# alibaba/easydist

Measured on AMD Instinct MI355X. Metric: gpt2_train_samples_per_sec, higher is better.
Workload: dtype bf16; 1 GPU; model=gpt2-small, global_batch=64, seq_len=1024, parallelism=auto(dp1)

## Files before the change

### easydist_amd/ops/csrc/gemm_kernels.hip

```cpp
#include "common.h"
#include "attn_block_map.h"
#include <torch/extension.h>
#include <ATen/cuda/CUDAContext.h>

using f32x4 = __attribute__((ext_vector_type(4))) float;
using bf16x8v = __attribute__((ext_vector_type(8))) __bf16;
using v4s = __attribute__((ext_vector_type(4))) short;
using v8s = __attribute__((ext_vector_type(8))) short;

DEVINL void glds16(const void* gsrc, void* lds_dst) {
  __builtin_amdgcn_global_load_lds(
      (const __attribute__((address_space(1))) unsigned int*)gsrc,
      (__attribute__((address_space(3))) unsigned int*)lds_dst, 16, 0, 0);
}

DEVINL void raw_barrier() { __builtin_amdgcn_s_barrier(); }

#define GELU_C 0.7978845608028654f
#define GELU_A 0.044715f

DEVINL float fast_tanh(float u) {
  return 1.f - 2.f / (__expf(2.f * u) + 1.f);
}

DEVINL float act_apply(int act, float x, float aux) {
  if (act == 1 || act == 3) {
    float u = GELU_C * (x + GELU_A * x * x * x);
    return 0.5f * x * (1.f + fast_tanh(u));
  }
  if (act == 2 || act == 4) {
    float u = GELU_C * (aux + GELU_A * aux * aux * aux);
    float t = fast_tanh(u);
    float d = 0.5f * (1.f + t)
              + 0.5f * aux * (1.f - t * t) * GELU_C
                    * (1.f + 3.f * GELU_A * aux * aux);
    return x * d;
  }
  if (act >= 5) {
    float u = GELU_C * (x + GELU_A * x * x * x);
    return 0.5f * x * (1.f + fast_tanh(u));
  }
  return x;
}

__global__ void __launch_bounds__(256)
gelu_fwd_kernel(const bf16* __restrict__ X, bf16* __restrict__ Y, long n) {
  long i = ((long)blockIdx.x * blockDim.x + threadIdx.x) * 8;
  for (; i + 7 < n; i += (long)gridDim.x * blockDim.x * 8) {
    bf16x8v x = *reinterpret_cast<const bf16x8v*>(&X[i]);
    bf16x8v y;
    #pragma unroll
    for (int e = 0; e < 8; ++e)
      y[e] = (__bf16)act_apply(1, bf2f((bf16)x[e]), 0.f);
    *reinterpret_cast<bf16x8v*>(&Y[i]) = y;
  }
}

__global__ void __launch_bounds__(256)
gelu_bwd_kernel(const bf16* __restrict__ G, const bf16* __restrict__ X,
                bf16* __restrict__ Y, long n) {
  long i = ((long)blockIdx.x * blockDim.x + threadIdx.x) * 8;
  for (; i + 7 < n; i += (long)gridDim.x * blockDim.x * 8) {
    bf16x8v g = *reinterpret_cast<const bf16x8v*>(&G[i]);
    bf16x8v x = *reinterpret_cast<const bf16x8v*>(&X[i]);
    bf16x8v y;
    #pragma unroll
    for (int e = 0; e < 8; ++e)
      y[e] = (__bf16)act_apply(2, bf2f((bf16)g[e]), bf2f((bf16)x[e]));
    *reinterpret_cast<bf16x8v*>(&Y[i]) = y;
  }
}

#define BM 128
#define BN 128
#define BK 32

extern "C" __global__ void __launch_bounds__(256)
gemm_nt_128(const bf16* __restrict__ A, const bf16* __restrict__ Bt,
            bf16* __restrict__ C, const bf16* __restrict__ bias,
            int M, int N, int K) {
  extern __shared__ __attribute__((aligned(16))) char smem[];
  const unsigned ATILE = BM * BK * 2;
  const unsigned BUF = 2 * ATILE;

  unsigned nwg_m = (M + BM - 1) / BM, nwg_n = (N + BN - 1) / BN;
  unsigned wg = xcd_swizzle(blockIdx.x, nwg_m * nwg_n);
  const unsigned m0 = (wg / nwg_n) * BM;
  const unsigned n0 = (wg % nwg_n) * BN;

  const int t = threadIdx.x;
  const int lane = t % WAVE;
  const int wave = t / WAVE;
  const int wm = (wave / 2) * 64;
  const int wn = (wave % 2) * 64;

  auto stage = [&](int buf, int k0) {
    #pragma unroll
    for (int p = 0; p < 2; ++p) {
      int e = (t + p * 256) * 8;
      int row = e / BK, col = e % BK;
      int grow = min((int)m0 + row, M - 1);
      const bf16* src = A + (long)grow * K + k0 + col;
      glds16(src, smem + buf * BUF + (p * 256 + wave * 64) * 16);
    }
    #pragma unroll
    for (int p = 0; p < 2; ++p) {
      int e = (t + p * 256) * 8;
      int row = e / BK, col = e % BK;
      int grow = min((int)n0 + row, N - 1);
      const bf16* src = Bt + (long)grow * K + k0 + col;
      glds16(src, smem + buf * BUF + ATILE + (p * 256 + wave * 64) * 16);
    }
  };

  f32x4 acc[4][4];
  #pragma unroll
  for (int i = 0; i < 4; ++i)
    #pragma unroll
    for (int j = 0; j < 4; ++j)
      acc[i][j] = {0.f, 0.f, 0.f, 0.f};

  stage(0, 0);
  __builtin_amdgcn_s_waitcnt(0);
  __syncthreads();

  const int frag_row = lane & 15;
  const int frag_k = (lane >> 4) * 8;

  int nk = K / BK;
  for (int kt = 0; kt < nk; ++kt) {
    int buf = kt & 1;
    if (kt + 1 < nk) stage(buf ^ 1, (kt + 1) * BK);
    bf16x8v a_frag[4], b_frag[4];
    const char* base = smem;
    #pragma unroll
    for (int i = 0; i < 4; ++i) {
      unsigned off = buf * BUF + ((wm + i * 16 + frag_row) * BK + frag_k) * 2;
      a_frag[i] = *reinterpret_cast<const bf16x8v*>(base + off);
    }
    #pragma unroll
    for (int j = 0; j < 4; ++j) {
      unsigned off = buf * BUF + ATILE +
                     ((wn + j * 16 + frag_row) * BK + frag_k) * 2;
      b_frag[j] = *reinterpret_cast<const bf16x8v*>(base + off);
    }
    #pragma unroll
    for (int i = 0; i < 4; ++i)
      #pragma unroll
      for (int j = 0; j < 4; ++j)
        acc[i][j] = __builtin_amdgcn_mfma_f32_16x16x32_bf16(
            a_frag[i], b_frag[j], acc[i][j], 0, 0, 0);
    __builtin_amdgcn_s_waitcnt(0);
    __syncthreads();
  }

  const int c_col = lane & 15;
  const int c_row0 = (lane >> 4) * 4;
  float bias_v[4] = {0.f, 0.f, 0.f, 0.f};
  if (bias) {
    #pragma unroll
    for (int j = 0; j < 4; ++j)
      bias_v[j] = bf2f(bias[min((int)(n0 + wn + j * 16 + c_col), N - 1)]);
  }
  #pragma unroll
  for (int i = 0; i < 4; ++i) {
    #pragma unroll
    for (int j = 0; j < 4; ++j) {
      #pragma unroll
      for (int reg = 0; reg < 4; ++reg) {
        int gm = m0 + wm + i * 16 + c_row0 + reg;
        int gn = n0 + wn + j * 16 + c_col;
        if (gm < M && gn < N)
          C[(long)gm * N + gn] = f2bf(acc[i][j][reg] + bias_v[j]);
      }
    }
  }
}

#define BM2 256
#define BN2 256
#define BK2 64
#define HALF_B 16384u
#define BUF_B 65536u

template <int SWZ>
DEVINL unsigned sw32(unsigned x) {
  if constexpr (SWZ == 0) return x ^ (((x >> 9) & 1u) << 5);
  else if constexpr (SWZ == 1) return x ^ (((x >> 9) & 3u) << 6);
  else return x ^ (((x >> 8) & 7u) << 4);
}

template <int SWZ>
__global__ void __launch_bounds__(512)
gemm_nt_256(const bf16* __restrict__ A, const bf16* __restrict__ Bt,
            bf16* __restrict__ C, const bf16* __restrict__ bias,
            bf16* __restrict__ aux, int act, int M, int N, int K) {
  extern __shared__ __attribute__((aligned(16))) char smem[];

  unsigned nwg_m = (M + BM2 - 1) / BM2, nwg_n = (N + BN2 - 1) / BN2;
  unsigned wg = xcd_swizzle(blockIdx.x, nwg_m * nwg_n);
  const unsigned m0 = (wg / nwg_n) * BM2;
  const unsigned n0 = (wg % nwg_n) * BN2;

  const int t = threadIdx.x;
  const int lane = t % WAVE;
  const int wave = t / WAVE;
  const int wr = wave >> 2;
  const int wc = wave & 3;

  auto stage_a = [&](int parity, int k0, int h) {
    unsigned dst0 = parity * BUF_B + h * HALF_B;
    #pragma unroll
    for (int i = 0; i < 2; ++i) {
      unsigned p = (i * 512 + t) * 16;
      unsigned L = sw32<SWZ>(p);
      int s = L >> 13;
      int row = (L >> 7) & 63;
      int k = (L & 127) >> 1;
      int grow = min((int)m0 + s * 128 + h * 64 + row, M - 1);
      glds16(A + (long)grow * K + k0 + k,
             smem + dst0 + (i * 512 + wave * 64) * 16);
    }
  };
  auto stage_b = [&](int parity, int k0, int h) {
    unsigned dst0 = parity * BUF_B + 32768u + h * HALF_B;
    #pragma unroll
    for (int i = 0; i < 2; ++i) {
      unsigned p = (i * 512 + t) * 16;
      unsigned L = sw32<SWZ>(p);
      int s = (L >> 12) & 3;
      int col = (L >> 7) & 31;
      int k = (L & 127) >> 1;
      int gcol = min((int)n0 + s * 64 + h * 32 + col, N - 1);
      glds16(Bt + (long)gcol * K + k0 + k,
             smem + dst0 + (i * 512 + wave * 64) * 16);
    }
  };

  const int fr = lane & 15;
  const int fg = lane >> 4;
  auto read_a = [&](bf16x8v (&a)[4][2], int tile, int mh) {
    unsigned base = (tile & 1) * BUF_B + mh * HALF_B;
    #pragma unroll
    for (int i = 0; i < 4; ++i)
      #pragma unroll
      for (int kk = 0; kk < 2; ++kk) {
        unsigned L = wr * 8192u + (i * 16 + fr) * 128u +
                     (kk * 32 + fg * 8) * 2u;
        a[i][kk] = *reinterpret_cast<const bf16x8v*>(smem + base + sw32<SWZ>(L));
      }
  };
  auto read_b = [&](bf16x8v (&b)[2][2], int tile, int nh) {
    unsigned base = (tile & 1) * BUF_B + 32768u + nh * HALF_B;
    #pragma unroll
    for (int j = 0; j < 2; ++j)
      #pragma unroll
      for (int kk = 0; kk < 2; ++kk) {
        unsigned L = wc * 4096u + (j * 16 + fr) * 128u +
                     (kk * 32 + fg * 8) * 2u;
        b[j][kk] = *reinterpret_cast<const bf16x8v*>(smem + base + sw32<SWZ>(L));
      }
  };

  f32x4 acc[8][4];
  #pragma unroll
  for (int i = 0; i < 8; ++i)
    #pragma unroll
    for (int j = 0; j < 4; ++j)
      acc[i][j] = {0.f, 0.f, 0.f, 0.f};

  bf16x8v a_frag[4][2], b_frag[2][2], b0_frag[2][2];
  const int NT = K / BK2;

  auto k_of = [&](int t) { return t < NT ? t * BK2 : 0; };

  stage_a(0, 0, 0); stage_a(0, 0, 1); stage_b(0, 0, 0); stage_b(0, 0, 1);
  stage_a(1, k_of(1), 0); stage_b(1, k_of(1), 1); stage_a(1, k_of(1), 1);
  asm volatile("s_waitcnt vmcnt(6)" ::: "memory");
  raw_barrier();

  auto mfma_quad = [&](int mh, int nh, bf16x8v (&bf)[2][2]) {
    __builtin_amdgcn_s_setprio(1);
    #pragma unroll
    for (int i = 0; i < 4; ++i)
      #pragma unroll
      for (int j = 0; j < 2; ++j)
        #pragma unroll
        for (int kk = 0; kk < 2; ++kk)
          acc[mh * 4 + i][nh * 2 + j] = __builtin_amdgcn_mfma_f32_16x16x32_bf16(
              a_frag[i][kk], bf[j][kk], acc[mh * 4 + i][nh * 2 + j],
              0, 0, 0);
    __builtin_amdgcn_s_setprio(0);
  };

  for (int T = 0; T < NT; ++T) {
    read_a(a_frag, T, 0);
    read_b(b0_frag, T, 0);
    read_b(b_frag, T, 1);
    stage_b((T + 1) & 1, k_of(T + 1), 0);
    mfma_quad(0, 0, b0_frag);
    raw_barrier();
    stage_a(T & 1, k_of(T + 2), 0);
    mfma_quad(0, 1, b_frag);
    raw_barrier();
    read_a(a_frag, T, 1);
    stage_b(T & 1, k_of(T + 2), 1);
    mfma_quad(1, 1, b_frag);
    raw_barrier();
    stage_a(T & 1, k_of(T + 2), 1);
    asm volatile("s_waitcnt vmcnt(6)" ::: "memory");
    mfma_quad(1, 0, b0_frag);
    raw_barrier();
  }

  asm volatile("s_waitcnt vmcnt(0)" ::: "memory");
  raw_barrier();
  bf16* share = reinterpret_cast<bf16*>(smem) + wave * 8192;
  const unsigned wm = wr * 128, wn = wc * 64;
  float bias_v[4] = {0.f, 0.f, 0.f, 0.f};
  if (bias) {
    #pragma unroll
    for (int j = 0; j < 4; ++j)
      bias_v[j] = bf2f(bias[min((int)(n0 + wn + j * 16 + fr), N - 1)]);
  }
  #pragma unroll
  for (int i = 0; i < 8; ++i)
    #pragma unroll
    for (int j = 0; j < 4; ++j)
      #pragma unroll
      for (int r = 0; r < 4; ++r) {
        int row = i * 16 + fg * 4 + r;
        int col = j * 16 + fr;
        share[row * 64 + col] = f2bf(acc[i][j][r] + bias_v[j]);
      }
  lds_fence();
  #pragma unroll
  for (int tt = 0; tt < 16; ++tt) {
    int row = tt * 8 + (lane >> 3);
    int colc = (lane & 7) * 8;
    int gm = m0 + wm + row;
    int gn = n0 + wn + colc;
    if (gm < (int)M && gn + 8 <= (int)N) {
      bf16x8v val = *reinterpret_cast<const bf16x8v*>(&share[row * 64 + colc]);
      if (act) {
        bf16x8v av{};
        if (act == 2 || act == 4)
          av = *reinterpret_cast<const bf16x8v*>(&aux[(long)gm * N + gn]);
        else if (act >= 5)
          *reinterpret_cast<bf16x8v*>(&aux[(long)gm * N + gn]) = val;
        #pragma unroll
        for (int e = 0; e < 8; ++e)
          val[e] = (__bf16)act_apply(act, bf2f((bf16)val[e]),
                                     bf2f((bf16)av[e]));
      }
      *reinterpret_cast<bf16x8v*>(&C[(long)gm * N + gn]) = val;
    } else if (gm < (int)M) {
      for (int e = 0; e < 8 && gn + e < (int)N; ++e) {
        float xv = bf2f(share[row * 64 + colc + e]);
        float axv = (act == 2 || act == 4)
                        ? bf2f(aux[(long)gm * N + gn + e]) : 0.f;
        if (act >= 5) aux[(long)gm * N + gn + e] = f2bf(xv);
        C[(long)gm * N + gn + e] = f2bf(act_apply(act, xv, axv));
      }
    }
  }
}

#define TBR 32
#define TBP 128

DEVINL int tn_unswz(int pos) { return ((pos >> 2) & 1) | ((pos & 3) << 1); }

DEVINL void tn_stage(const bf16* src, long ld, int r0, int p0, int pmax,
                     char* dst_base, int t, int wave) {
  #pragma unroll
  for (int i = 0; i < 2; ++i) {
    unsigned p = (i * 256 + t) * 16;
    int chunk16 = p >> 10;
    unsigned w = p & 1023u;
    int bpos = w >> 7;
    int blk = tn_unswz(bpos);
    int rr = blk * 4 + ((w & 127) >> 5);
    int pp = chunk16 * 16 + ((w & 31) >> 1);
    int gp = min(p0 + pp, pmax - 8);
    glds16(src + (long)(r0 + rr) * ld + gp,
           dst_base + (i * 256 + wave * 64) * 16);
  }
}

DEVINL bf16x8v tn_frag(const char* img, int chunk, int lane) {
  const char* base = img + chunk * 1024 + (lane >> 4) * 128 + (lane & 15) * 8;
  v4s lo = __builtin_amdgcn_ds_read_tr16_b64_v4i16(
      (__attribute__((address_space(3))) v4s*)base);
  v4s hi = __builtin_amdgcn_ds_read_tr16_b64_v4i16(
      (__attribute__((address_space(3))) v4s*)(base + 512));
  v8s out = __builtin_shufflevector(lo, hi, 0, 1, 2, 3, 4, 5, 6, 7);
  return __builtin_bit_cast(bf16x8v, out);
}

extern "C" __global__ void __launch_bounds__(256)
gemm_tn_kernel(const bf16* __restrict__ Ag, const bf16* __restrict__ Bg,
               float* __restrict__ Cw, float* __restrict__ Asum,
               int R, int P, int Q, int splitr) {
  extern __shared__ __attribute__((aligned(16))) char smem[];
  const unsigned IMG = TBR * TBP * 2;
  const unsigned BUF = 2 * IMG;

  unsigned nwg_p = P / TBP, nwg_q = Q / TBP;
  unsigned ntile = nwg_p * nwg_q;
  unsigned wg = xcd_swizzle(blockIdx.x, ntile * splitr);
  unsigned tile = wg / splitr, slice = wg % splitr;
  const unsigned p0 = (tile / nwg_q) * TBP;
  const unsigned q0 = (tile % nwg_q) * TBP;

  int nrt_all = R / TBR;
  int per = (nrt_all + splitr - 1) / splitr;
  int rt0 = slice * per;
  int rt1 = min(nrt_all, rt0 + per);
  if (rt0 >= rt1) return;

  const int t = threadIdx.x;
  const int lane = t % WAVE;
  const int wave = t / WAVE;
  const int wp = (wave >> 1) * 64;
  const int wq = (wave & 1) * 64;

  auto stage = [&](int buf, int rt) {
    tn_stage(Ag, P, rt * TBR, p0, P, smem + buf * BUF, t, wave);
    tn_stage(Bg, Q, rt * TBR, q0, Q, smem + buf * BUF + IMG, t, wave);
  };

  f32x4 acc[4][4];
  float asum_acc[4] = {0.f, 0.f, 0.f, 0.f};
  #pragma unroll
  for (int i = 0; i < 4; ++i)
    #pragma unroll
    for (int j = 0; j < 4; ++j)
      acc[i][j] = {0.f, 0.f, 0.f, 0.f};

  stage(0, rt0);
  __builtin_amdgcn_s_waitcnt(0);
  __syncthreads();
  for (int rt = rt0; rt < rt1; ++rt) {
    int buf = (rt - rt0) & 1;
    if (rt + 1 < rt1) stage(buf ^ 1, rt + 1);
    bf16x8v a_frag[4], b_frag[4];
    #pragma unroll
    for (int i = 0; i < 4; ++i)
      a_frag[i] = tn_frag(smem + buf * BUF, (wp >> 4) + i, lane);
    if (Asum && q0 == 0 && (wave & 1) == 0) {
      #pragma unroll
      for (int i = 0; i < 4; ++i) {
        float acc_s = 0.f;
        #pragma unroll
        for (int u = 0; u < 8; ++u) acc_s += bf2f((bf16)a_frag[i][u]);
        asum_acc[i] += acc_s;
      }
    }
    #pragma unroll
    for (int j = 0; j < 4; ++j)
      b_frag[j] = tn_frag(smem + buf * BUF + IMG, (wq >> 4) + j, lane);
    #pragma unroll
    for (int i = 0; i < 4; ++i)
      #pragma unroll
      for (int j = 0; j < 4; ++j)
        acc[i][j] = __builtin_amdgcn_mfma_f32_16x16x32_bf16(
            a_frag[i], b_frag[j], acc[i][j], 0, 0, 0);
    __builtin_amdgcn_s_waitcnt(0);
    __syncthreads();
  }

  if (Asum && q0 == 0 && (wave & 1) == 0) {
    #pragma unroll
    for (int i = 0; i < 4; ++i) {
      float v = asum_acc[i];
      v += __shfl_down(v, 32, WAVE);
      v += __shfl_down(v, 16, WAVE);
      if (lane < 16) {
        int gp = p0 + wp + i * 16 + lane;
        if (gp < P) atomicAdd(&Asum[gp], v);
      }
    }
  }
  const int c_col = lane & 15;
  const int c_row0 = (lane >> 4) * 4;
  #pragma unroll
  for (int i = 0; i < 4; ++i)
    #pragma unroll
    for (int j = 0; j < 4; ++j)
      #pragma unroll
      for (int reg = 0; reg < 4; ++reg) {
        int gp = p0 + wp + i * 16 + c_row0 + reg;
        int gq = q0 + wq + j * 16 + c_col;
        if (gp < P && gq < Q) {
          if (splitr == 1)
            Cw[(long)gp * Q + gq] = acc[i][j][reg];
          else
            atomicAdd(&Cw[(long)gp * Q + gq], acc[i][j][reg]);
        }
      }
}

#define TBP2 256

DEVINL void tn_stage2(const bf16* src, long ld, int r0, int p0, int pmax,
                      char* dst_base, int t, int wave) {
  #pragma unroll
  for (int i = 0; i < 2; ++i) {
    unsigned p = (i * 512 + t) * 16;
    int chunk16 = p >> 10;
    unsigned w = p & 1023u;
    int bpos = w >> 7;
    int blk = tn_unswz(bpos);
    int rr = blk * 4 + ((w & 127) >> 5);
    int pp = chunk16 * 16 + ((w & 31) >> 1);
    int gp = min(p0 + pp, pmax - 8);
    glds16(src + (long)(r0 + rr) * ld + gp,
           dst_base + (i * 512 + wave * 64) * 16);
  }
}

extern "C" __global__ void __launch_bounds__(512)
gemm_tn_256_kernel(const bf16* __restrict__ Ag, const bf16* __restrict__ Bg,
                   float* __restrict__ Cw, float* __restrict__ Asum,
                   int R, int P, int Q, int splitr) {
  extern __shared__ __attribute__((aligned(16))) char smem[];
  const unsigned IMG = TBR * TBP2 * 2;
  const unsigned BUF = 2 * IMG;

  unsigned nwg_p = (P + TBP2 - 1) / TBP2, nwg_q = (Q + TBP2 - 1) / TBP2;
  unsigned ntile = nwg_p * nwg_q;
  unsigned wg = xcd_swizzle(blockIdx.x, ntile * splitr);
  unsigned tile = wg / splitr, slice = wg % splitr;
  const unsigned p0 = (tile / nwg_q) * TBP2;
  const unsigned q0 = (tile % nwg_q) * TBP2;

  int nrt_all = R / TBR;
  int per = (nrt_all + splitr - 1) / splitr;
  int rt0 = slice * per;
  int rt1 = min(nrt_all, rt0 + per);
  if (rt0 >= rt1) return;

  const int t = threadIdx.x;
  const int lane = t % WAVE;
  const int wave = t / WAVE;
  const int wp = (wave >> 1) * 64;
  const int wq = (wave & 1) * 128;

  auto stage = [&](int buf, int rt) {
    tn_stage2(Ag, P, rt * TBR, p0, P, smem + buf * BUF, t, wave);
    tn_stage2(Bg, Q, rt * TBR, q0, Q, smem + buf * BUF + IMG, t, wave);
  };

  f32x4 acc[4][8];
  float asum_acc[4] = {0.f, 0.f, 0.f, 0.f};
  #pragma unroll
  for (int i = 0; i < 4; ++i)
    #pragma unroll
    for (int j = 0; j < 8; ++j)
      acc[i][j] = {0.f, 0.f, 0.f, 0.f};

  stage(0, rt0);
  __builtin_amdgcn_s_waitcnt(0);
  __syncthreads();
  for (int rt = rt0; rt < rt1; ++rt) {
    int buf = (rt - rt0) & 1;
    if (rt + 1 < rt1) stage(buf ^ 1, rt + 1);
    bf16x8v a_frag[4], b_frag[8];
    #pragma unroll
    for (int i = 0; i < 4; ++i)
      a_frag[i] = tn_frag(smem + buf * BUF, (wp >> 4) + i, lane);
    if (Asum && q0 == 0 && (wave & 1) == 0) {
      #pragma unroll
      for (int i = 0; i < 4; ++i) {
        float acc_s = 0.f;
        #pragma unroll
        for (int u = 0; u < 8; ++u) acc_s += bf2f((bf16)a_frag[i][u]);
        asum_acc[i] += acc_s;
      }
    }
    #pragma unroll
    for (int j = 0; j < 8; ++j)
      b_frag[j] = tn_frag(smem + buf * BUF + IMG, (wq >> 4) + j, lane);
    #pragma unroll
    for (int i = 0; i < 4; ++i)
      #pragma unroll
      for (int j = 0; j < 8; ++j)
        acc[i][j] = __builtin_amdgcn_mfma_f32_16x16x32_bf16(
            a_frag[i], b_frag[j], acc[i][j], 0, 0, 0);
    __builtin_amdgcn_s_waitcnt(0);
    __syncthreads();
  }

  if (Asum && q0 == 0 && (wave & 1) == 0) {
    #pragma unroll
    for (int i = 0; i < 4; ++i) {
      float v = asum_acc[i];
      v += __shfl_down(v, 32, WAVE);
      v += __shfl_down(v, 16, WAVE);
      if (lane < 16) {
        int gp = p0 + wp + i * 16 + lane;
        if (gp < P) atomicAdd(&Asum[gp], v);
      }
    }
  }
  const int c_col = lane & 15;
  const int c_row0 = (lane >> 4) * 4;
  #pragma unroll
  for (int i = 0; i < 4; ++i)
    #pragma unroll
    for (int j = 0; j < 8; ++j)
      #pragma unroll
      for (int reg = 0; reg < 4; ++reg) {
        int gp = p0 + wp + i * 16 + c_row0 + reg;
        int gq = q0 + wq + j * 16 + c_col;
        if (gp < P && gq < Q) {
          if (splitr == 1)
            Cw[(long)gp * Q + gq] = acc[i][j][reg];
          else
            atomicAdd(&Cw[(long)gp * Q + gq], acc[i][j][reg]);
        }
      }
}

at::Tensor gemm_nt_act(const at::Tensor& a, const at::Tensor& bt,
                       const std::optional<at::Tensor>& bias, int64_t act,
                       const std::optional<at::Tensor>& aux) {
  TORCH_CHECK(a.dtype() == at::kBFloat16 && bt.dtype() == at::kBFloat16);
  TORCH_CHECK(a.is_contiguous() && bt.is_contiguous(),
              "gemm_nt wants K-contiguous operands");
  const long M = a.size(0), K = a.size(1), N = bt.size(0);
  TORCH_CHECK(bt.size(1) == K);
  TORCH_CHECK(K % BK == 0, "gemm_nt: K must be a multiple of 32");
  TORCH_CHECK(N % 8 == 0, "gemm_nt: N must be a multiple of 8");
  auto c = at::empty({M, N}, a.options());
  auto stream = at::cuda::getCurrentCUDAStream();
  const bf16* bias_p = bias ? (const bf16*)bias->data_ptr() : nullptr;
  if (K % BK2 == 0 && M >= BM2 && N >= 128) {
    unsigned nwg = ((M + BM2 - 1) / BM2) * ((N + BN2 - 1) / BN2);
    static int swz = []() {
      const char* e = getenv("EASYDIST_NT256_SWZ");
      return e ? atoi(e) : 2;
    }();
    auto kern = swz == 0 ? gemm_nt_256<0> : swz == 2 ? gemm_nt_256<2>
                                          : gemm_nt_256<1>;
    bf16* aux_p = aux ? (bf16*)aux->data_ptr() : nullptr;
    TORCH_CHECK(act == 0 || !(act >= 2) || aux_p,
                "gemm_nt: activation modes 2/4/5/6 need aux");
    hipLaunchKernelGGL(kern, dim3(nwg), dim3(512), 2 * BUF_B, stream,
        (const bf16*)a.data_ptr(), (const bf16*)bt.data_ptr(),
        (bf16*)c.data_ptr(), bias_p, aux_p, (int)act, (int)M, (int)N,
        (int)K);
  } else {
    unsigned nwg = ((M + BM - 1) / BM) * ((N + BN - 1) / BN);
    size_t lds = 2 * 2 * BM * BK * 2;
    hipLaunchKernelGGL(gemm_nt_128, dim3(nwg), dim3(256), lds, stream,
        (const bf16*)a.data_ptr(), (const bf16*)bt.data_ptr(),
        (bf16*)c.data_ptr(), bias_p, (int)M, (int)N, (int)K);
    if (act) {
      if (act == 1) c = at::gelu(c, "tanh");
      else if (act == 3) c = at::gelu(c);
      else if (act == 2) c = at::gelu_backward(c, aux.value(), "tanh");
      else if (act == 4) c = at::gelu_backward(c, aux.value(), "none");
      else if (act >= 5) {
        aux.value().copy_(c);
        c = at::gelu(c, "tanh");
      }
    }
  }
  return c;
}

at::Tensor gemm_nt(const at::Tensor& a, const at::Tensor& bt,
                   const std::optional<at::Tensor>& bias) {
  return gemm_nt_act(a, bt, bias, 0, std::nullopt);
}

at::Tensor gelu_fast(const at::Tensor& x) {
  TORCH_CHECK(x.dtype() == at::kBFloat16 && x.is_contiguous());
  const long n = x.numel();
  TORCH_CHECK(n % 8 == 0, "gelu_fast: numel multiple of 8");
  auto y = at::empty_like(x);
  long thr = n / 8;
  unsigned grid = (unsigned)std::min<long>((thr + 255) / 256, 8192);
  auto stream = at::cuda::getCurrentCUDAStream();
  hipLaunchKernelGGL(gelu_fwd_kernel, dim3(grid), dim3(256), 0, stream,
                     (const bf16*)x.data_ptr(), (bf16*)y.data_ptr(), n);
  return y;
}

at::Tensor gelu_bwd_fast(const at::Tensor& g, const at::Tensor& x) {
  TORCH_CHECK(g.dtype() == at::kBFloat16 && g.is_contiguous());
  TORCH_CHECK(x.dtype() == at::kBFloat16 && x.is_contiguous());
  const long n = x.numel();
  TORCH_CHECK(g.numel() == n && n % 8 == 0);
  auto y = at::empty_like(x);
  long thr = n / 8;
  unsigned grid = (unsigned)std::min<long>((thr + 255) / 256, 8192);
  auto stream = at::cuda::getCurrentCUDAStream();
  hipLaunchKernelGGL(gelu_bwd_kernel, dim3(grid), dim3(256), 0, stream,
                     (const bf16*)g.data_ptr(), (const bf16*)x.data_ptr(),
                     (bf16*)y.data_ptr(), n);
  return y;
}

std::tuple<at::Tensor, at::Tensor>
gemm_nt_gelu(const at::Tensor& a, const at::Tensor& bt,
             const std::optional<at::Tensor>& bias, bool tanh_approx) {
  const long M = a.size(0), K = a.size(1), N = bt.size(0);
  if (K % BK2 == 0 && M >= BM2 && N >= 128) {
    auto pre = at::empty({M, N}, a.options());
    auto act = gemm_nt_act(a, bt, bias, tanh_approx ? 5 : 6, pre);
    return {act, pre};
  }
  auto pre = gemm_nt_act(a, bt, bias, 0, std::nullopt);
  auto act = at::gelu(pre, tanh_approx ? "tanh" : "none");
  return {act, pre};
}

std::tuple<at::Tensor, at::Tensor> gemm_tn_asum(const at::Tensor& a,
                                                const at::Tensor& b);

static at::Tensor tn_launch(const at::Tensor& a, const at::Tensor& b,
                            float* asum_p) {
  TORCH_CHECK(a.dtype() == at::kBFloat16 && b.dtype() == at::kBFloat16);
  TORCH_CHECK(a.is_contiguous() && b.is_contiguous());
  const long R = a.size(0), P = a.size(1), Q = b.size(0) == R ? b.size(1) : -1;
  TORCH_CHECK(Q > 0, "gemm_tn: reduce dims must match");
  TORCH_CHECK(R % TBR == 0, "gemm_tn: R must be a multiple of 32");
  TORCH_CHECK(P % TBP == 0 && Q % TBP == 0,
              "gemm_tn: P, Q must be multiples of 128");
  static int use256 = []() {
    const char* e = getenv("EASYDIST_TN256");
    return e ? atoi(e) : 1;
  }();
  bool big = use256 && R / TBR >= 64 && P >= TBP2 && Q >= TBP2;
  unsigned ntile;
  int splitr = 1;
  if (big) {
    ntile = ((P + TBP2 - 1) / TBP2) * ((Q + TBP2 - 1) / TBP2);
    static int target = []() {
      const char* e = getenv("EASYDIST_TN256_TARGET");
      return e ? atoi(e) : 256;
    }();
    splitr = std::max(1, target / (int)ntile);
    splitr = std::min((long)splitr, R / TBR / 8);
    splitr = std::max(1, std::min(splitr, 64));
  } else {
    ntile = (P / TBP) * (Q / TBP);
    while (ntile * splitr < 512 && splitr < 16 &&
           (R / TBR) % (splitr * 2) == 0 && (R / TBR) / (splitr * 2) >= 1)
      splitr *= 2;
  }
  auto cw = splitr == 1
      ? at::empty({P, Q}, a.options().dtype(at::kFloat))
      : at::zeros({P, Q}, a.options().dtype(at::kFloat));
  auto stream = at::cuda::getCurrentCUDAStream();
  if (big) {
    size_t lds = 2 * 2 * TBR * TBP2 * 2;
    hipLaunchKernelGGL(gemm_tn_256_kernel, dim3(ntile * splitr), dim3(512),
        lds, stream,
        (const bf16*)a.data_ptr(), (const bf16*)b.data_ptr(),
        cw.data_ptr<float>(), asum_p, (int)R, (int)P, (int)Q, splitr);
  } else {
    size_t lds = 2 * 2 * TBR * TBP * 2;
    hipLaunchKernelGGL(gemm_tn_kernel, dim3(ntile * splitr), dim3(256), lds,
        stream,
        (const bf16*)a.data_ptr(), (const bf16*)b.data_ptr(),
        cw.data_ptr<float>(), asum_p, (int)R, (int)P, (int)Q, splitr);
  }
  return cw;
}

at::Tensor gemm_tn(const at::Tensor& a, const at::Tensor& b) {
  return tn_launch(a, b, nullptr).to(at::kBFloat16);
}

std::tuple<at::Tensor, at::Tensor> gemm_tn_asum(const at::Tensor& a,
                                                const at::Tensor& b) {
  auto asum = at::zeros({a.size(1)}, a.options().dtype(at::kFloat));
  auto cw = tn_launch(a, b, asum.data_ptr<float>());
  return {cw.to(at::kBFloat16), asum};
}
```

### easydist_amd/ops/csrc/norm_kernels.hip

```cpp
#include "common.h"
#include <string>
#include <cstdlib>

template <typename T, bool RMS>
__global__ void norm_fwd_kernel(const T* __restrict__ x,
                                const T* __restrict__ w,
                                const T* __restrict__ b,
                                T* __restrict__ out,
                                float* __restrict__ mean_out,
                                float* __restrict__ rstd_out,
                                int rows, int D, float eps) {
  const int wave_id = (blockIdx.x * blockDim.x + threadIdx.x) / WAVE;
  const int lane = threadIdx.x % WAVE;
  if (wave_id >= rows) return;
  const T* xrow = x + (long)wave_id * D;
  T* orow = out + (long)wave_id * D;

  const int VEC = 8;
  float s1 = 0.f, s2 = 0.f;
  for (int i = lane * VEC; i < D; i += WAVE * VEC) {
    bf16x8 xv = *reinterpret_cast<const bf16x8*>(&xrow[i]);
    #pragma unroll
    for (int j = 0; j < VEC; ++j) {
      float f = bf2f(xv.v[j]);
      s1 += f;
      s2 += f * f;
    }
  }
  s1 = wave_sum(s1);
  s2 = wave_sum(s2);
  float mean, rstd;
  if (RMS) {
    mean = 0.f;
    rstd = rsqrtf(s2 / D + eps);
  } else {
    mean = s1 / D;
    rstd = rsqrtf(fmaxf(s2 / D - mean * mean, 0.f) + eps);
  }
  if (lane == 0) {
    if (!RMS) mean_out[wave_id] = mean;
    rstd_out[wave_id] = rstd;
  }
  for (int i = lane * VEC; i < D; i += WAVE * VEC) {
    bf16x8 xv = *reinterpret_cast<const bf16x8*>(&xrow[i]);
    bf16x8 ov;
    bf16x8 wv, bv;
    if (w) wv = *reinterpret_cast<const bf16x8*>(&w[i]);
    if (b) bv = *reinterpret_cast<const bf16x8*>(&b[i]);
    #pragma unroll
    for (int j = 0; j < VEC; ++j) {
      float f = (bf2f(xv.v[j]) - mean) * rstd;
      if (w) f *= bf2f(wv.v[j]);
      if (b) f += bf2f(bv.v[j]);
      ov.v[j] = f2bf(f);
    }
    *reinterpret_cast<bf16x8*>(&orow[i]) = ov;
  }
}

template <bool RMS>
__global__ void norm_fwd_kernel_f32(const float* __restrict__ x,
                                    const float* __restrict__ w,
                                    const float* __restrict__ b,
                                    float* __restrict__ out,
                                    float* __restrict__ mean_out,
                                    float* __restrict__ rstd_out,
                                    int rows, int D, float eps) {
  const int wave_id = (blockIdx.x * blockDim.x + threadIdx.x) / WAVE;
  const int lane = threadIdx.x % WAVE;
  if (wave_id >= rows) return;
  const float* xrow = x + (long)wave_id * D;
  float* orow = out + (long)wave_id * D;
  const int VEC = 4;
  float s1 = 0.f, s2 = 0.f;
  for (int i = lane * VEC; i < D; i += WAVE * VEC) {
    float4 xv = *reinterpret_cast<const float4*>(&xrow[i]);
    s1 += xv.x + xv.y + xv.z + xv.w;
    s2 += xv.x * xv.x + xv.y * xv.y + xv.z * xv.z + xv.w * xv.w;
  }
  s1 = wave_sum(s1);
  s2 = wave_sum(s2);
  float mean, rstd;
  if (RMS) {
    mean = 0.f;
    rstd = rsqrtf(s2 / D + eps);
  } else {
    mean = s1 / D;
    rstd = rsqrtf(fmaxf(s2 / D - mean * mean, 0.f) + eps);
  }
  if (lane == 0) {
    if (!RMS) mean_out[wave_id] = mean;
    rstd_out[wave_id] = rstd;
  }
  for (int i = lane * VEC; i < D; i += WAVE * VEC) {
    float4 xv = *reinterpret_cast<const float4*>(&xrow[i]);
    float4 ov;
    float* xp = &xv.x;
    float* op = &ov.x;
    #pragma unroll
    for (int j = 0; j < VEC; ++j) {
      float f = (xp[j] - mean) * rstd;
      if (w) f *= w[i + j];
      if (b) f += b[i + j];
      op[j] = f;
    }
    *reinterpret_cast<float4*>(&orow[i]) = ov;
  }
}

template <typename T, bool RMS>
__global__ void norm_bwd_kernel(const T* __restrict__ grad,
                                const T* __restrict__ x,
                                const float* __restrict__ mean,
                                const float* __restrict__ rstd,
                                const T* __restrict__ w,
                                T* __restrict__ dx,
                                float* __restrict__ dw,
                                float* __restrict__ db,
                                int rows, int D) {
  const int wave_id = (blockIdx.x * blockDim.x + threadIdx.x) / WAVE;
  const int lane = threadIdx.x % WAVE;
  if (wave_id >= rows) return;
  const T* grow = grad + (long)wave_id * D;
  const T* xrow = x + (long)wave_id * D;
  T* dxrow = dx + (long)wave_id * D;
  const float m = RMS ? 0.f : mean[wave_id];
  const float r = rstd[wave_id];

  const int VEC = 8;
  float sum_gw = 0.f, sum_gwx = 0.f;
  for (int i = lane * VEC; i < D; i += WAVE * VEC) {
    bf16x8 gv = *reinterpret_cast<const bf16x8*>(&grow[i]);
    bf16x8 xv = *reinterpret_cast<const bf16x8*>(&xrow[i]);
    bf16x8 wv;
    if (w) wv = *reinterpret_cast<const bf16x8*>(&w[i]);
    #pragma unroll
    for (int j = 0; j < VEC; ++j) {
      float g = bf2f(gv.v[j]);
      float xh = (bf2f(xv.v[j]) - m) * r;
      float gw = w ? g * bf2f(wv.v[j]) : g;
      sum_gw += gw;
      sum_gwx += gw * xh;
    }
  }
  sum_gw = wave_sum(sum_gw) / D;
  sum_gwx = wave_sum(sum_gwx) / D;
  for (int i = lane * VEC; i < D; i += WAVE * VEC) {
    bf16x8 gv = *reinterpret_cast<const bf16x8*>(&grow[i]);
    bf16x8 xv = *reinterpret_cast<const bf16x8*>(&xrow[i]);
    bf16x8 wv;
    if (w) wv = *reinterpret_cast<const bf16x8*>(&w[i]);
    bf16x8 dxv;
    #pragma unroll
    for (int j = 0; j < VEC; ++j) {
      float g = bf2f(gv.v[j]);
      float xh = (bf2f(xv.v[j]) - m) * r;
      float gw = w ? g * bf2f(wv.v[j]) : g;
      float v = RMS ? r * (gw - xh * sum_gwx)
                    : r * (gw - sum_gw - xh * sum_gwx);
      dxv.v[j] = f2bf(v);
    }
    *reinterpret_cast<bf16x8*>(&dxrow[i]) = dxv;
  }
}

template <typename T, bool RMS>
__global__ void norm_param_grads_kernel(const T* __restrict__ grad,
                                        const T* __restrict__ x,
                                        const float* __restrict__ mean,
                                        const float* __restrict__ rstd,
                                        float* __restrict__ dw,
                                        float* __restrict__ db,
                                        int rows, int D, int rows_per_blk) {
  const int col0 = (blockIdx.x * blockDim.x + threadIdx.x) * 8;
  if (col0 >= D) return;
  const int r0 = blockIdx.y * rows_per_blk;
  const int r1 = min(r0 + rows_per_blk, rows);
  float sw[8] = {0, 0, 0, 0, 0, 0, 0, 0};
  float sb[8] = {0, 0, 0, 0, 0, 0, 0, 0};
  for (int r = r0; r < r1; ++r) {
    const bf16x8 g8 = *reinterpret_cast<const bf16x8*>(
        &grad[(long)r * D + col0]);
    const bf16x8 x8 = *reinterpret_cast<const bf16x8*>(
        &x[(long)r * D + col0]);
    const float m = RMS ? 0.f : mean[r];
    const float rs = rstd[r];
    #pragma unroll
    for (int u = 0; u < 8; ++u) {
      float g = bf2f(g8.v[u]);
      sw[u] += g * (bf2f(x8.v[u]) - m) * rs;
      sb[u] += g;
    }
  }
  #pragma unroll
  for (int u = 0; u < 8; ++u) {
    atomicAdd(&dw[col0 + u], sw[u]);
    atomicAdd(&db[col0 + u], sb[u]);
  }
}

template <typename T, bool RMS>
__global__ void norm_param_grads_scalar_kernel(const T* __restrict__ grad,
                                               const T* __restrict__ x,
                                               const float* __restrict__ mean,
                                               const float* __restrict__ rstd,
                                               float* __restrict__ dw,
                                               float* __restrict__ db,
                                               int rows, int D,
                                               int rows_per_blk) {
  const int col = blockIdx.x * blockDim.x + threadIdx.x;
  if (col >= D) return;
  const int r0 = blockIdx.y * rows_per_blk;
  const int r1 = min(r0 + rows_per_blk, rows);
  float sw = 0.f, sb = 0.f;
  #pragma unroll 8
  for (int r = r0; r < r1; ++r) {
    float g = bf2f(grad[(long)r * D + col]);
    float m = RMS ? 0.f : mean[r];
    float xh = (bf2f(x[(long)r * D + col]) - m) * rstd[r];
    sw += g * xh;
    sb += g;
  }
  atomicAdd(&dw[col], sw);
  atomicAdd(&db[col], sb);
}

static bool lnpg_scalar() {
  static int v = [] {
    const char* e = getenv("EASYDIST_LNPG");
    return (e && std::string(e) == "vector") ? 0 : 1;
  }();
  return v;
}

#include <torch/extension.h>
#include <ATen/cuda/CUDAContext.h>

static void check_lastdim(const at::Tensor& x) {
  TORCH_CHECK(x.is_contiguous(), "norm kernels need contiguous input");
  TORCH_CHECK(x.size(-1) % 8 == 0, "feature dim must be a multiple of 8");
}

static void check_affine(const at::Tensor& x,
                         const std::optional<at::Tensor>& w,
                         const std::optional<at::Tensor>& b) {
  if (w) TORCH_CHECK(w->numel() == x.size(-1), "weight/feature mismatch");
  if (b) TORCH_CHECK(b->numel() == x.size(-1), "bias/feature mismatch");
}

std::tuple<at::Tensor, at::Tensor, at::Tensor>
layer_norm_fwd(const at::Tensor& x, const std::optional<at::Tensor>& w,
               const std::optional<at::Tensor>& b, double eps) {
  check_lastdim(x);
  check_affine(x, w, b);
  const int D = x.size(-1);
  const long rows = x.numel() / D;
  auto out = at::empty_like(x);
  auto stat_shape = x.sizes().vec();
  stat_shape.back() = 1;
  auto mean = at::empty(stat_shape, x.options().dtype(at::kFloat));
  auto rstd = at::empty(stat_shape, x.options().dtype(at::kFloat));
  auto stream = at::cuda::getCurrentCUDAStream();
  const int WPB = 4;
  dim3 block(WAVE * WPB), grid((rows + WPB - 1) / WPB);
  if (x.scalar_type() == at::kBFloat16) {
    hipLaunchKernelGGL((norm_fwd_kernel<bf16, false>), grid, block, 0, stream,
        (const bf16*)x.data_ptr(), w ? (const bf16*)w->data_ptr() : nullptr,
        b ? (const bf16*)b->data_ptr() : nullptr, (bf16*)out.data_ptr(),
        mean.data_ptr<float>(), rstd.data_ptr<float>(), rows, D, (float)eps);
  } else {
    hipLaunchKernelGGL((norm_fwd_kernel_f32<false>), grid, block, 0, stream,
        x.data_ptr<float>(), w ? w->data_ptr<float>() : nullptr,
        b ? b->data_ptr<float>() : nullptr, out.data_ptr<float>(),
        mean.data_ptr<float>(), rstd.data_ptr<float>(), rows, D, (float)eps);
  }
  return {out, mean, rstd};
}

std::tuple<at::Tensor, at::Tensor, at::Tensor>
layer_norm_bwd(const at::Tensor& grad, const at::Tensor& x,
               const at::Tensor& mean, const at::Tensor& rstd,
               const std::optional<at::Tensor>& w,
               std::vector<bool> mask) {
  check_lastdim(x);
  check_affine(x, w, std::nullopt);
  TORCH_CHECK(grad.sizes() == x.sizes() && grad.is_contiguous());
  TORCH_CHECK(mean.numel() == x.numel() / x.size(-1));
  TORCH_CHECK(x.scalar_type() == at::kBFloat16,
              "layer_norm_bwd kernel: bf16 only (fp32 falls back to aten)");
  const int D = x.size(-1);
  const long rows = x.numel() / D;
  auto dx = at::empty_like(x);
  auto dwf = at::zeros({D}, x.options().dtype(at::kFloat));
  auto dbf = at::zeros({D}, x.options().dtype(at::kFloat));
  auto stream = at::cuda::getCurrentCUDAStream();
  const int WPB = 4;
  dim3 block(WAVE * WPB), grid((rows + WPB - 1) / WPB);
  hipLaunchKernelGGL((norm_bwd_kernel<bf16, false>), grid, block, 0, stream,
      (const bf16*)grad.data_ptr(), (const bf16*)x.data_ptr(),
      mean.data_ptr<float>(), rstd.data_ptr<float>(),
      w ? (const bf16*)w->data_ptr() : nullptr, (bf16*)dx.data_ptr(),
      dwf.data_ptr<float>(), dbf.data_ptr<float>(), rows, D);
  const int gx = (D + 511) / 512;
  int rows_per_blk = 256;
  while ((long)gx * ((rows + rows_per_blk - 1) / rows_per_blk) > 1024)
    rows_per_blk *= 2;
  dim3 gblock(64), ggrid(gx, (rows + rows_per_blk - 1) / rows_per_blk);
  if (lnpg_scalar()) {
    const int rpb2 = 256;
    dim3 sb2(256), sg2((D + 255) / 256, (rows + rpb2 - 1) / rpb2);
    hipLaunchKernelGGL((norm_param_grads_scalar_kernel<bf16, false>), sg2,
        sb2, 0, stream, (const bf16*)grad.data_ptr(),
        (const bf16*)x.data_ptr(), mean.data_ptr<float>(),
        rstd.data_ptr<float>(), dwf.data_ptr<float>(),
        dbf.data_ptr<float>(), rows, D, rpb2);
    auto dtype0 = at::kFloat;
    return {dx, dwf.to(dtype0), dbf.to(dtype0)};
  }
  hipLaunchKernelGGL((norm_param_grads_kernel<bf16, false>), ggrid, gblock, 0,
      stream, (const bf16*)grad.data_ptr(), (const bf16*)x.data_ptr(),
      mean.data_ptr<float>(), rstd.data_ptr<float>(), dwf.data_ptr<float>(),
      dbf.data_ptr<float>(), rows, D, rows_per_blk);
  auto dtype = at::kFloat;
  return {dx, dwf.to(dtype), dbf.to(dtype)};
}

std::tuple<at::Tensor, at::Tensor>
rms_norm_fwd(const at::Tensor& x, const std::optional<at::Tensor>& w,
             double eps) {
  check_lastdim(x);
  check_affine(x, w, std::nullopt);
  const int D = x.size(-1);
  const long rows = x.numel() / D;
  auto out = at::empty_like(x);
  auto stat_shape = x.sizes().vec();
  stat_shape.back() = 1;
  auto rstd = at::empty(stat_shape, x.options().dtype(at::kFloat));
  auto stream = at::cuda::getCurrentCUDAStream();
  const int WPB = 4;
  dim3 block(WAVE * WPB), grid((rows + WPB - 1) / WPB);
  if (x.scalar_type() == at::kBFloat16) {
    hipLaunchKernelGGL((norm_fwd_kernel<bf16, true>), grid, block, 0, stream,
        (const bf16*)x.data_ptr(), w ? (const bf16*)w->data_ptr() : nullptr,
        nullptr, (bf16*)out.data_ptr(), nullptr, rstd.data_ptr<float>(),
        rows, D, (float)eps);
  } else {
    hipLaunchKernelGGL((norm_fwd_kernel_f32<true>), grid, block, 0, stream,
        x.data_ptr<float>(), w ? w->data_ptr<float>() : nullptr, nullptr,
        out.data_ptr<float>(), nullptr, rstd.data_ptr<float>(), rows, D,
        (float)eps);
  }
  return {out, rstd};
}

std::tuple<at::Tensor, at::Tensor>
rms_norm_bwd(const at::Tensor& grad, const at::Tensor& x,
             const at::Tensor& rstd, const std::optional<at::Tensor>& w) {
  check_lastdim(x);
  check_affine(x, w, std::nullopt);
  TORCH_CHECK(grad.sizes() == x.sizes() && grad.is_contiguous());
  TORCH_CHECK(x.scalar_type() == at::kBFloat16, "rms_norm_bwd: bf16 only");
  const int D = x.size(-1);
  const long rows = x.numel() / D;
  auto dx = at::empty_like(x);
  auto dwf = at::zeros({D}, x.options().dtype(at::kFloat));
  auto dbf = at::zeros({D}, x.options().dtype(at::kFloat));
  auto stream = at::cuda::getCurrentCUDAStream();
  const int WPB = 4;
  dim3 block(WAVE * WPB), grid((rows + WPB - 1) / WPB);
  hipLaunchKernelGGL((norm_bwd_kernel<bf16, true>), grid, block, 0, stream,
      (const bf16*)grad.data_ptr(), (const bf16*)x.data_ptr(), nullptr,
      rstd.data_ptr<float>(), w ? (const bf16*)w->data_ptr() : nullptr,
      (bf16*)dx.data_ptr(), dwf.data_ptr<float>(), dbf.data_ptr<float>(),
      rows, D);
  const int gx = (D + 511) / 512;
  int rows_per_blk = 256;
  while ((long)gx * ((rows + rows_per_blk - 1) / rows_per_blk) > 1024)
    rows_per_blk *= 2;
  dim3 gblock(64), ggrid(gx, (rows + rows_per_blk - 1) / rows_per_blk);
  hipLaunchKernelGGL((norm_param_grads_kernel<bf16, true>), ggrid, gblock, 0,
      stream, (const bf16*)grad.data_ptr(), (const bf16*)x.data_ptr(),
      nullptr, rstd.data_ptr<float>(), dwf.data_ptr<float>(),
      dbf.data_ptr<float>(), rows, D, rows_per_blk);
  auto dtype = at::kFloat;
  return {dx, dwf.to(dtype)};
}
```

### easydist_amd/ops/csrc/optim_kernels.hip

```cpp
#include "common.h"
#include <torch/extension.h>
#include <ATen/cuda/CUDAContext.h>
#include <ATen/cuda/CUDAGraphsUtils.cuh>
#include <map>
#include <utility>
#include <vector>

struct AdamChunk {
  const float* p;
  const void* g;
  const float* ea;
  const float* eas;
  float* out_p;
  float* out_ea;
  float* out_eas;
  int tensor_idx;
  int n;
};

DEVINL void load_g4(const void* g, int i, int g_bf16, float* out) {
  if (g_bf16) {
    bf16x8 v = *reinterpret_cast<const bf16x8*>(&((const bf16*)g)[i & ~7]);
    const int o = i & 4;
    #pragma unroll
    for (int j = 0; j < 4; ++j) out[j] = bf2f(v.v[o + j]);
  } else {
    float4 v = *reinterpret_cast<const float4*>(&((const float*)g)[i]);
    out[0] = v.x; out[1] = v.y; out[2] = v.z; out[3] = v.w;
  }
}

#define CHUNK_ELEMS 65536

struct StagingPair {
  at::Tensor pinned, dev;
  size_t capacity = 0;
  hipEvent_t h2d_done = nullptr;
};

static StagingPair& staging_for(std::map<std::pair<size_t, const void*>,
                                         StagingPair>& pool,
                                size_t bytes, const void* key_ptr,
                                const at::Device& dev, bool capturing,
                                const char* who) {
  auto& st = pool[{bytes, key_ptr}];
  if (bytes > st.capacity) {
    TORCH_CHECK(!capturing, who,
                ": staging buffers must be warmed up (one eager call per "
                "parameter bank) before hipGraph capture");
    st.pinned = at::empty({(long)bytes},
                          at::TensorOptions().dtype(at::kByte)
                              .pinned_memory(true));
    st.dev = at::empty({(long)bytes},
                       at::TensorOptions().dtype(at::kByte).device(dev));
    st.capacity = bytes;
  }
  if (st.h2d_done == nullptr)
    C10_CUDA_CHECK(hipEventCreateWithFlags(&st.h2d_done,
                                           hipEventDisableTiming));
  else if (!capturing)
    C10_CUDA_CHECK(hipEventSynchronize(st.h2d_done));
  return st;
}

static void staging_finish(std::map<std::pair<size_t, const void*>,
                                    StagingPair>& pool,
                           size_t bytes, const void* key_ptr,
                           bool capturing, hipStream_t stream) {
  auto it = pool.find({bytes, key_ptr});
  if (it == pool.end()) return;
  if (capturing) {
    static std::vector<at::Tensor> keepalive;
    keepalive.push_back(it->second.pinned);
    keepalive.push_back(it->second.dev);
    pool.erase(it);
  } else {
    C10_CUDA_CHECK(hipEventRecord(it->second.h2d_done, stream));
  }
}

__global__ void fused_adam_kernel(const AdamChunk* __restrict__ chunks,
                                  int n_chunks, int g_bf16,
                                  const float* __restrict__ steps,
                                  float lr, float beta1, float beta2,
                                  float weight_decay, float eps) {
  const int c = blockIdx.x;
  if (c >= n_chunks) return;
  const AdamChunk ch = chunks[c];
  const float step = steps[ch.tensor_idx] + 1.f;
  const float bc1 = 1.f - __powf(beta1, step);
  const float bc2 = 1.f - __powf(beta2, step);
  const float inv_bc1 = 1.f / bc1;
  const float rsqrt_bc2 = rsqrtf(bc2);
  #pragma unroll 4
  for (int i = threadIdx.x * 4; i + 3 < ch.n; i += blockDim.x * 4) {
    float4 p = *reinterpret_cast<const float4*>(&ch.p[i]);
    float gg[4];
    load_g4(ch.g, i, g_bf16, gg);
    float4 ea = *reinterpret_cast<const float4*>(&ch.ea[i]);
    float4 eas = *reinterpret_cast<const float4*>(&ch.eas[i]);
    float* pp = &p.x; float* ee = &ea.x; float* ss = &eas.x;
    #pragma unroll
    for (int j = 0; j < 4; ++j) {
      float grad = gg[j];
      if (weight_decay != 0.f) grad += weight_decay * pp[j];
      float m = beta1 * ee[j] + (1.f - beta1) * grad;
      float v = beta2 * ss[j] + (1.f - beta2) * grad * grad;
      float denom = __fsqrt_rn(v) * rsqrt_bc2 + eps;
      pp[j] = pp[j] - lr * (m * inv_bc1) / denom;
      ee[j] = m;
      ss[j] = v;
    }
    *reinterpret_cast<float4*>(&ch.out_p[i]) = p;
    *reinterpret_cast<float4*>(&ch.out_ea[i]) = ea;
    *reinterpret_cast<float4*>(&ch.out_eas[i]) = eas;
  }
  int tail_start = (ch.n / 4) * 4;
  for (int i = tail_start + threadIdx.x; i < ch.n; i += blockDim.x) {
    float grad = g_bf16 ? bf2f(((const bf16*)ch.g)[i])
                        : ((const float*)ch.g)[i];
    if (weight_decay != 0.f) grad += weight_decay * ch.p[i];
    float m = beta1 * ch.ea[i] + (1.f - beta1) * grad;
    float v = beta2 * ch.eas[i] + (1.f - beta2) * grad * grad;
    float denom = __fsqrt_rn(v) * rsqrt_bc2 + eps;
    ch.out_p[i] = ch.p[i] - lr * (m * inv_bc1) / denom;
    ch.out_ea[i] = m;
    ch.out_eas[i] = v;
  }
}

__global__ void bump_steps_kernel(const float* const* __restrict__ in_steps,
                                  float* const* __restrict__ out_steps,
                                  int n) {
  int i = blockIdx.x * blockDim.x + threadIdx.x;
  if (i < n) out_steps[i][0] = in_steps[i][0] + 1.f;
}

std::tuple<std::vector<at::Tensor>, std::vector<at::Tensor>,
           std::vector<at::Tensor>, std::vector<at::Tensor>>
fused_adam_step(std::vector<at::Tensor> params, std::vector<at::Tensor> grads,
                std::vector<at::Tensor> exp_avgs,
                std::vector<at::Tensor> exp_avg_sqs,
                std::vector<at::Tensor> steps, double lr, double beta1,
                double beta2, double weight_decay, double eps) {
  const int T = params.size();
  std::vector<at::Tensor> out_p, out_ea, out_eas, out_steps;
  out_p.reserve(T); out_ea.reserve(T); out_eas.reserve(T);
  const bool g_bf16 = !grads.empty()
      && grads[0].scalar_type() == at::kBFloat16;
  for (int t = 0; t < T; ++t) {
    TORCH_CHECK(params[t].scalar_type() == at::kFloat, "fp32 params only");
    TORCH_CHECK(grads[t].scalar_type()
                    == (g_bf16 ? at::kBFloat16 : at::kFloat),
                "grads must be uniformly fp32 or bf16");
    TORCH_CHECK(params[t].is_contiguous() && grads[t].is_contiguous());
    out_p.push_back(at::empty_like(params[t]));
    out_ea.push_back(at::empty_like(exp_avgs[t]));
    out_eas.push_back(at::empty_like(exp_avg_sqs[t]));
    out_steps.push_back(at::empty_like(steps[t]));
  }
  auto steps_flat = at::empty({T}, params[0].options());
  {
    std::vector<at::Tensor> svec;
    for (auto& s : steps) svec.push_back(s.reshape({1}).to(at::kFloat));
    at::cat_out(steps_flat, svec, 0);
  }

  std::vector<AdamChunk> chunks;
  for (int t = 0; t < T; ++t) {
    long n = params[t].numel();
    for (long off = 0; off < n; off += CHUNK_ELEMS) {
      AdamChunk c;
      c.p = params[t].data_ptr<float>() + off;
      c.g = g_bf16 ? (const void*)((const bf16*)grads[t].data_ptr() + off)
                   : (const void*)(grads[t].data_ptr<float>() + off);
      c.ea = exp_avgs[t].data_ptr<float>() + off;
      c.eas = exp_avg_sqs[t].data_ptr<float>() + off;
      c.out_p = out_p[t].data_ptr<float>() + off;
      c.out_ea = out_ea[t].data_ptr<float>() + off;
      c.out_eas = out_eas[t].data_ptr<float>() + off;
      c.tensor_idx = t;
      c.n = (int)std::min<long>(CHUNK_ELEMS, n - off);
      chunks.push_back(c);
    }
  }
  static std::map<std::pair<size_t, const void*>, StagingPair> g_pool;
  const size_t bytes = chunks.size() * sizeof(AdamChunk);
  const void* key = params[0].data_ptr();
  bool capturing = at::cuda::currentStreamCaptureStatusMayInitCtx() !=
                   at::cuda::CaptureStatus::None;
  auto& st = staging_for(g_pool, bytes, key, params[0].device(), capturing,
                         "fused_adam_step");
  memcpy(st.pinned.data_ptr(), chunks.data(), bytes);
  auto stream = at::cuda::getCurrentCUDAStream();
  C10_CUDA_CHECK(hipMemcpyAsync(st.dev.data_ptr(), st.pinned.data_ptr(),
                                bytes, hipMemcpyHostToDevice, stream));
  hipLaunchKernelGGL(fused_adam_kernel, dim3(chunks.size()), dim3(256), 0,
      stream, (const AdamChunk*)st.dev.data_ptr(), (int)chunks.size(),
      (int)g_bf16, steps_flat.data_ptr<float>(), (float)lr, (float)beta1,
      (float)beta2, (float)weight_decay, (float)eps);
  staging_finish(g_pool, bytes, key, capturing, stream);
  for (int t = 0; t < T; ++t)
    out_steps[t] = steps[t] + 1;
  return {out_p, out_ea, out_eas, out_steps};
}

struct SgdChunk {
  const float* p;
  const void* g;
  const float* buf;
  float* out_p;
  float* out_buf;
  int n;
};

__global__ void fused_sgd_kernel(const SgdChunk* __restrict__ chunks,
                                 int n_chunks, int g_bf16, float lr,
                                 float momentum, float dampening,
                                 float weight_decay, int nesterov) {
  const int c = blockIdx.x;
  if (c >= n_chunks) return;
  const SgdChunk ch = chunks[c];
  for (int i = threadIdx.x; i < ch.n; i += blockDim.x) {
    float grad = g_bf16 ? bf2f(((const bf16*)ch.g)[i])
                        : ((const float*)ch.g)[i];
    if (weight_decay != 0.f) grad += weight_decay * ch.p[i];
    float upd = grad;
    if (momentum != 0.f) {
      float nb = momentum * ch.buf[i] + (1.f - dampening) * grad;
      ch.out_buf[i] = nb;
      upd = nesterov ? grad + momentum * nb : nb;
    }
    ch.out_p[i] = ch.p[i] - lr * upd;
  }
}

std::tuple<std::vector<at::Tensor>, std::vector<at::Tensor>>
fused_sgd_step(std::vector<at::Tensor> params, std::vector<at::Tensor> grads,
               std::vector<at::Tensor> bufs, double lr, double momentum,
               double dampening, double weight_decay, bool nesterov) {
  const int T = params.size();
  const bool has_m = momentum != 0.0;
  TORCH_CHECK(!has_m || (int)bufs.size() == T,
              "momentum needs one buffer per param");
  std::vector<at::Tensor> out_p, out_buf;
  out_p.reserve(T);
  const bool g_bf16 = !grads.empty()
      && grads[0].scalar_type() == at::kBFloat16;
  for (int t = 0; t < T; ++t) {
    TORCH_CHECK(params[t].scalar_type() == at::kFloat, "fp32 params only");
    TORCH_CHECK(grads[t].scalar_type()
                    == (g_bf16 ? at::kBFloat16 : at::kFloat),
                "grads must be uniformly fp32 or bf16");
    TORCH_CHECK(params[t].is_contiguous() && grads[t].is_contiguous());
    out_p.push_back(at::empty_like(params[t]));
    if (has_m) out_buf.push_back(at::empty_like(bufs[t]));
  }
  std::vector<SgdChunk> chunks;
  for (int t = 0; t < T; ++t) {
    long n = params[t].numel();
    for (long off = 0; off < n; off += CHUNK_ELEMS) {
      SgdChunk c;
      c.p = params[t].data_ptr<float>() + off;
      c.g = g_bf16 ? (const void*)((const bf16*)grads[t].data_ptr() + off)
                   : (const void*)(grads[t].data_ptr<float>() + off);
      c.buf = has_m ? bufs[t].data_ptr<float>() + off : nullptr;
      c.out_p = out_p[t].data_ptr<float>() + off;
      c.out_buf = has_m ? out_buf[t].data_ptr<float>() + off : nullptr;
      c.n = (int)std::min<long>(CHUNK_ELEMS, n - off);
      chunks.push_back(c);
    }
  }
  static std::map<std::pair<size_t, const void*>, StagingPair> g_pool;
  const size_t bytes = chunks.size() * sizeof(SgdChunk);
  const void* key = params[0].data_ptr();
  bool capturing = at::cuda::currentStreamCaptureStatusMayInitCtx() !=
                   at::cuda::CaptureStatus::None;
  auto& st = staging_for(g_pool, bytes, key, params[0].device(), capturing,
                         "fused_sgd_step");
  memcpy(st.pinned.data_ptr(), chunks.data(), bytes);
  auto stream = at::cuda::getCurrentCUDAStream();
  C10_CUDA_CHECK(hipMemcpyAsync(st.dev.data_ptr(), st.pinned.data_ptr(),
                                bytes, hipMemcpyHostToDevice, stream));
  hipLaunchKernelGGL(fused_sgd_kernel, dim3(chunks.size()), dim3(256), 0,
      stream, (const SgdChunk*)st.dev.data_ptr(), (int)chunks.size(),
      (int)g_bf16, (float)lr, (float)momentum, (float)dampening,
      (float)weight_decay, nesterov ? 1 : 0);
  staging_finish(g_pool, bytes, key, capturing, stream);
  return {out_p, out_buf};
}
```

Before: 727.5 samples/sec.

## Fuse bf16 output into TN GEMM, rewrite norm backward, fold step bump into Adam

The TN GEMM now writes bf16 output directly when not split. Split-R runs accumulate into a persistent fp32 workspace, and a small finish kernel converts it to bf16 and re-zeroes it. This removes the fp32 allocation plus zeros and the separate .to(bf16) pass. Layer/RMS-norm backward is restructured into a persistent 1024-thread kernel that computes dx and accumulates weight/bias grads in LDS in one pass, replacing the separate param-grad kernels. Adam now reads and writes step counters inside the fused kernel, dropping the cat of the step tensors and the per-tensor add launches. The cost is more complex code and workspace state that must stay safe under graph capture.

```diff
diff --git a/easydist_amd/ops/csrc/gemm_kernels.hip b/easydist_amd/ops/csrc/gemm_kernels.hip
--- a/easydist_amd/ops/csrc/gemm_kernels.hip
+++ b/easydist_amd/ops/csrc/gemm_kernels.hip
@@ -2,6 +2,11 @@
 #include "attn_block_map.h"
 #include <torch/extension.h>
 #include <ATen/cuda/CUDAContext.h>
+#include <ATen/cuda/CUDAGraphsUtils.cuh>
+#include <map>
+#include <mutex>
+#include <utility>
+#include <vector>
 
 using f32x4 = __attribute__((ext_vector_type(4))) float;
 using bf16x8v = __attribute__((ext_vector_type(8))) __bf16;
@@ -398,10 +403,85 @@
   return __builtin_bit_cast(bf16x8v, out);
 }
 
+struct TnOut {
+  bf16* C;
+  float* asum;
+  float* ws;
+  float* ws_asum;
+};
+
+template <int NJ>
+DEVINL void tn_epilogue(f32x4 (&acc)[4][NJ], const float (&asum_acc)[4],
+                        const TnOut& o, int P, int Q, unsigned p0,
+                        unsigned q0, int wp, int wq, int nslices) {
+  const int lane = threadIdx.x % WAVE;
+  const int wave = threadIdx.x / WAVE;
+  const bool direct = nslices == 1;
+
+  if (o.asum && q0 == 0 && (wave & 1) == 0) {
+    #pragma unroll
+    for (int i = 0; i < 4; ++i) {
+      float v = asum_acc[i];
+      v += __shfl_down(v, 32, WAVE);
+      v += __shfl_down(v, 16, WAVE);
+      if (lane < 16) {
+        int gp = p0 + wp + i * 16 + lane;
+        if (gp < P) {
+          if (direct) o.asum[gp] = v;
+          else atomicAdd(&o.ws_asum[gp], v);
+        }
+      }
+    }
+  }
+  const int c_col = lane & 15;
+  const int c_row0 = (lane >> 4) * 4;
+  #pragma unroll
+  for (int i = 0; i < 4; ++i)
+    #pragma unroll
+    for (int j = 0; j < NJ; ++j)
+      #pragma unroll
+      for (int reg = 0; reg < 4; ++reg) {
+        int gp = p0 + wp + i * 16 + c_row0 + reg;
+        int gq = q0 + wq + j * 16 + c_col;
+        if (gp < P && gq < Q) {
+          if (direct)
+            o.C[(long)gp * Q + gq] = f2bf(acc[i][j][reg]);
+          else
+            atomicAdd(&o.ws[(long)gp * Q + gq], acc[i][j][reg]);
+        }
+      }
+}
+
+__global__ void __launch_bounds__(256)
+tn_finish_kernel(float* __restrict__ ws, bf16* __restrict__ C, long n,
+                 float* __restrict__ ws_asum, float* __restrict__ asum,
+                 int P) {
+  const long tid = (long)blockIdx.x * blockDim.x + threadIdx.x;
+  const long stride = (long)gridDim.x * blockDim.x;
+  const float4 zero4 = {0.f, 0.f, 0.f, 0.f};
+  for (long g = tid; g < n / 8; g += stride) {
+    float4* src = reinterpret_cast<float4*>(ws + g * 8);
+    const float4 lo = src[0], hi = src[1];
+    src[0] = zero4;
+    src[1] = zero4;
+    bf16x8 out;
+    out.v[0] = f2bf(lo.x); out.v[1] = f2bf(lo.y);
+    out.v[2] = f2bf(lo.z); out.v[3] = f2bf(lo.w);
+    out.v[4] = f2bf(hi.x); out.v[5] = f2bf(hi.y);
+    out.v[6] = f2bf(hi.z); out.v[7] = f2bf(hi.w);
+    *reinterpret_cast<bf16x8*>(C + g * 8) = out;
+  }
+  if (asum) {
+    for (long p = tid; p < P; p += stride) {
+      asum[p] = ws_asum[p];
+      ws_asum[p] = 0.f;
+    }
+  }
+}
+
 extern "C" __global__ void __launch_bounds__(256)
 gemm_tn_kernel(const bf16* __restrict__ Ag, const bf16* __restrict__ Bg,
-               float* __restrict__ Cw, float* __restrict__ Asum,
-               int R, int P, int Q, int splitr) {
+               TnOut out, int R, int P, int Q, int splitr) {
   extern __shared__ __attribute__((aligned(16))) char smem[];
   const unsigned IMG = TBR * TBP * 2;
   const unsigned BUF = 2 * IMG;
@@ -417,6 +497,7 @@
   int per = (nrt_all + splitr - 1) / splitr;
   int rt0 = slice * per;
   int rt1 = min(nrt_all, rt0 + per);
+  const int nslices = (nrt_all + per - 1) / per;
   if (rt0 >= rt1) return;
 
   const int t = threadIdx.x;
@@ -448,7 +529,7 @@
     #pragma unroll
     for (int i = 0; i < 4; ++i)
       a_frag[i] = tn_frag(smem + buf * BUF, (wp >> 4) + i, lane);
-    if (Asum && q0 == 0 && (wave & 1) == 0) {
+    if (out.asum && q0 == 0 && (wave & 1) == 0) {
       #pragma unroll
       for (int i = 0; i < 4; ++i) {
         float acc_s = 0.f;
@@ -470,35 +551,7 @@
     __syncthreads();
   }
 
-  if (Asum && q0 == 0 && (wave & 1) == 0) {
-    #pragma unroll
-    for (int i = 0; i < 4; ++i) {
-      float v = asum_acc[i];
-      v += __shfl_down(v, 32, WAVE);
-      v += __shfl_down(v, 16, WAVE);
-      if (lane < 16) {
-        int gp = p0 + wp + i * 16 + lane;
-        if (gp < P) atomicAdd(&Asum[gp], v);
-      }
-    }
-  }
-  const int c_col = lane & 15;
-  const int c_row0 = (lane >> 4) * 4;
-  #pragma unroll
-  for (int i = 0; i < 4; ++i)
-    #pragma unroll
-    for (int j = 0; j < 4; ++j)
-      #pragma unroll
-      for (int reg = 0; reg < 4; ++reg) {
-        int gp = p0 + wp + i * 16 + c_row0 + reg;
-        int gq = q0 + wq + j * 16 + c_col;
-        if (gp < P && gq < Q) {
-          if (splitr == 1)
-            Cw[(long)gp * Q + gq] = acc[i][j][reg];
-          else
-            atomicAdd(&Cw[(long)gp * Q + gq], acc[i][j][reg]);
-        }
-      }
+  tn_epilogue<4>(acc, asum_acc, out, P, Q, p0, q0, wp, wq, nslices);
 }
 
 #define TBP2 256
@@ -522,8 +575,7 @@
 
 extern "C" __global__ void __launch_bounds__(512)
 gemm_tn_256_kernel(const bf16* __restrict__ Ag, const bf16* __restrict__ Bg,
-                   float* __restrict__ Cw, float* __restrict__ Asum,
-                   int R, int P, int Q, int splitr) {
+                   TnOut out, int R, int P, int Q, int splitr) {
   extern __shared__ __attribute__((aligned(16))) char smem[];
   const unsigned IMG = TBR * TBP2 * 2;
   const unsigned BUF = 2 * IMG;
@@ -539,6 +591,7 @@
   int per = (nrt_all + splitr - 1) / splitr;
   int rt0 = slice * per;
   int rt1 = min(nrt_all, rt0 + per);
+  const int nslices = (nrt_all + per - 1) / per;
   if (rt0 >= rt1) return;
 
   const int t = threadIdx.x;
@@ -570,7 +623,7 @@
     #pragma unroll
     for (int i = 0; i < 4; ++i)
       a_frag[i] = tn_frag(smem + buf * BUF, (wp >> 4) + i, lane);
-    if (Asum && q0 == 0 && (wave & 1) == 0) {
+    if (out.asum && q0 == 0 && (wave & 1) == 0) {
       #pragma unroll
       for (int i = 0; i < 4; ++i) {
         float acc_s = 0.f;
@@ -592,35 +645,7 @@
     __syncthreads();
   }
 
-  if (Asum && q0 == 0 && (wave & 1) == 0) {
-    #pragma unroll
-    for (int i = 0; i < 4; ++i) {
-      float v = asum_acc[i];
-      v += __shfl_down(v, 32, WAVE);
-      v += __shfl_down(v, 16, WAVE);
-      if (lane < 16) {
-        int gp = p0 + wp + i * 16 + lane;
-        if (gp < P) atomicAdd(&Asum[gp], v);
-      }
-    }
-  }
-  const int c_col = lane & 15;
-  const int c_row0 = (lane >> 4) * 4;
-  #pragma unroll
-  for (int i = 0; i < 4; ++i)
-    #pragma unroll
-    for (int j = 0; j < 8; ++j)
-      #pragma unroll
-      for (int reg = 0; reg < 4; ++reg) {
-        int gp = p0 + wp + i * 16 + c_row0 + reg;
-        int gq = q0 + wq + j * 16 + c_col;
-        if (gp < P && gq < Q) {
-          if (splitr == 1)
-            Cw[(long)gp * Q + gq] = acc[i][j][reg];
-          else
-            atomicAdd(&Cw[(long)gp * Q + gq], acc[i][j][reg]);
-        }
-      }
+  tn_epilogue<8>(acc, asum_acc, out, P, Q, p0, q0, wp, wq, nslices);
 }
 
 at::Tensor gemm_nt_act(const at::Tensor& a, const at::Tensor& bt,
@@ -721,6 +746,28 @@
 std::tuple<at::Tensor, at::Tensor> gemm_tn_asum(const at::Tensor& a,
                                                 const at::Tensor& b);
 
+struct TnWorkspace {
+  at::Tensor ws;
+  long cap = 0;
+  bool captured = false;
+};
+
+static float* tn_workspace(const at::Tensor& like, hipStream_t stream,
+                           long need, bool capturing) {
+  static std::mutex mu;
+  static std::map<std::pair<int, hipStream_t>, TnWorkspace> pool;
+  static std::vector<at::Tensor> keepalive;
+  std::lock_guard<std::mutex> lock(mu);
+  auto& w = pool[{(int)like.get_device(), stream}];
+  if (need > w.cap) {
+    if (w.captured) keepalive.push_back(w.ws);
+    w.ws = at::zeros({need}, like.options().dtype(at::kFloat));
+    w.cap = need;
+  }
+  if (capturing) w.captured = true;
+  return w.ws.data_ptr<float>();
+}
+
 static at::Tensor tn_launch(const at::Tensor& a, const at::Tensor& b,
                             float* asum_p) {
   TORCH_CHECK(a.dtype() == at::kBFloat16 && b.dtype() == at::kBFloat16);
@@ -752,33 +799,45 @@
            (R / TBR) % (splitr * 2) == 0 && (R / TBR) / (splitr * 2) >= 1)
       splitr *= 2;
   }
-  auto cw = splitr == 1
-      ? at::empty({P, Q}, a.options().dtype(at::kFloat))
-      : at::zeros({P, Q}, a.options().dtype(at::kFloat));
+  auto c = at::empty({P, Q}, a.options());
   auto stream = at::cuda::getCurrentCUDAStream();
+  TnOut out{(bf16*)c.data_ptr(), asum_p, nullptr, nullptr};
+  if (splitr > 1) {
+    const bool capturing = at::cuda::currentStreamCaptureStatusMayInitCtx() !=
+                           at::cuda::CaptureStatus::None;
+    out.ws = tn_workspace(a, stream.stream(), P * Q + (asum_p ? P : 0),
+                          capturing);
+    out.ws_asum = asum_p ? out.ws + P * Q : nullptr;
+  }
   if (big) {
     size_t lds = 2 * 2 * TBR * TBP2 * 2;
     hipLaunchKernelGGL(gemm_tn_256_kernel, dim3(ntile * splitr), dim3(512),
         lds, stream,
-        (const bf16*)a.data_ptr(), (const bf16*)b.data_ptr(),
-        cw.data_ptr<float>(), asum_p, (int)R, (int)P, (int)Q, splitr);
+        (const bf16*)a.data_ptr(), (const bf16*)b.data_ptr(), out,
+        (int)R, (int)P, (int)Q, splitr);
   } else {
     size_t lds = 2 * 2 * TBR * TBP * 2;
     hipLaunchKernelGGL(gemm_tn_kernel, dim3(ntile * splitr), dim3(256), lds,
         stream,
-        (const bf16*)a.data_ptr(), (const bf16*)b.data_ptr(),
-        cw.data_ptr<float>(), asum_p, (int)R, (int)P, (int)Q, splitr);
-  }
-  return cw;
+        (const bf16*)a.data_ptr(), (const bf16*)b.data_ptr(), out,
+        (int)R, (int)P, (int)Q, splitr);
+  }
+  if (splitr > 1) {
+    const long n = P * Q;
+    unsigned grid = (unsigned)std::min<long>((n / 8 + 255) / 256, 2048);
+    hipLaunchKernelGGL(tn_finish_kernel, dim3(grid), dim3(256), 0, stream,
+        out.ws, out.C, n, out.ws_asum, out.asum, (int)P);
+  }
+  return c;
 }
 
 at::Tensor gemm_tn(const at::Tensor& a, const at::Tensor& b) {
-  return tn_launch(a, b, nullptr).to(at::kBFloat16);
+  return tn_launch(a, b, nullptr);
 }
 
 std::tuple<at::Tensor, at::Tensor> gemm_tn_asum(const at::Tensor& a,
                                                 const at::Tensor& b) {
-  auto asum = at::zeros({a.size(1)}, a.options().dtype(at::kFloat));
-  auto cw = tn_launch(a, b, asum.data_ptr<float>());
-  return {cw.to(at::kBFloat16), asum};
-}
+  auto asum = at::empty({a.size(1)}, a.options().dtype(at::kFloat));
+  auto c = tn_launch(a, b, asum.data_ptr<float>());
+  return {c, asum};
+}
diff --git a/easydist_amd/ops/csrc/norm_kernels.hip b/easydist_amd/ops/csrc/norm_kernels.hip
--- a/easydist_amd/ops/csrc/norm_kernels.hip
+++ b/easydist_amd/ops/csrc/norm_kernels.hip
@@ -1,5 +1,5 @@
 #include "common.h"
-#include <string>
+#include <algorithm>
 #include <cstdlib>
 
 template <typename T, bool RMS>
@@ -108,129 +108,163 @@
   }
 }
 
-template <typename T, bool RMS>
-__global__ void norm_bwd_kernel(const T* __restrict__ grad,
-                                const T* __restrict__ x,
-                                const float* __restrict__ mean,
-                                const float* __restrict__ rstd,
-                                const T* __restrict__ w,
-                                T* __restrict__ dx,
-                                float* __restrict__ dw,
-                                float* __restrict__ db,
-                                int rows, int D) {
-  const int wave_id = (blockIdx.x * blockDim.x + threadIdx.x) / WAVE;
+#define NORM_BWD_THREADS 1024
+#define NORM_VEC 8
+#define NORM_CSTRIDE (WAVE * NORM_VEC)
+
+DEVINL int norm_red_slot(int col8, int j, int D8) { return j * D8 + (col8 >> 3); }
+
+DEVINL void norm_opaque(bf16x8& v) {
+  using u32x4 = __attribute__((ext_vector_type(4))) unsigned;
+  u32x4 u = __builtin_bit_cast(u32x4, v);
+  asm volatile("" : "+v"(u));
+  v = __builtin_bit_cast(bf16x8, u);
+}
+
+template <bool RMS>
+DEVINL void norm_row_sums(const bf16x8& gv, const bf16x8& xv,
+                          const bf16x8& wv, bool has_w, float m, float r,
+                          float& sum_gw, float& sum_gwx) {
+  #pragma unroll
+  for (int j = 0; j < NORM_VEC; ++j) {
+    float g = bf2f(gv.v[j]);
+    float xh = (bf2f(xv.v[j]) - m) * r;
+    float gw = has_w ? g * bf2f(wv.v[j]) : g;
+    sum_gw += gw;
+    sum_gwx += gw * xh;
+  }
+}
+
+template <bool RMS>
+DEVINL bf16x8 norm_row_dx(const bf16x8& gv, const bf16x8& xv,
+                          const bf16x8& wv, bool has_w, float m, float r,
+                          float sum_gw, float sum_gwx, float* sw, float* sb) {
+  bf16x8 dxv;
+  #pragma unroll
+  for (int j = 0; j < NORM_VEC; ++j) {
+    float g = bf2f(gv.v[j]);
+    float xh = (bf2f(xv.v[j]) - m) * r;
+    float gw = has_w ? g * bf2f(wv.v[j]) : g;
+    float v = RMS ? r * (gw - xh * sum_gwx)
+                  : r * (gw - sum_gw - xh * sum_gwx);
+    dxv.v[j] = f2bf(v);
+    sw[j] += g * xh;
+    if (!RMS) sb[j] += g;
+  }
+  return dxv;
+}
+
+template <typename T, bool RMS, int NC>
+__global__ void __launch_bounds__(NORM_BWD_THREADS)
+norm_bwd_kernel(const T* __restrict__ grad,
+                const T* __restrict__ x,
+                const float* __restrict__ mean,
+                const float* __restrict__ rstd,
+                const T* __restrict__ w,
+                T* __restrict__ dx,
+                float* __restrict__ dwb,
+                int rows, int D) {
+  extern __shared__ float red[];
+  const int nred = (RMS ? 1 : 2) * D;
+  for (int c = threadIdx.x; c < nred; c += blockDim.x) red[c] = 0.f;
+  __syncthreads();
+
   const int lane = threadIdx.x % WAVE;
-  if (wave_id >= rows) return;
-  const T* grow = grad + (long)wave_id * D;
-  const T* xrow = x + (long)wave_id * D;
-  T* dxrow = dx + (long)wave_id * D;
-  const float m = RMS ? 0.f : mean[wave_id];
-  const float r = rstd[wave_id];
-
-  const int VEC = 8;
-  float sum_gw = 0.f, sum_gwx = 0.f;
-  for (int i = lane * VEC; i < D; i += WAVE * VEC) {
-    bf16x8 gv = *reinterpret_cast<const bf16x8*>(&grow[i]);
-    bf16x8 xv = *reinterpret_cast<const bf16x8*>(&xrow[i]);
-    bf16x8 wv;
-    if (w) wv = *reinterpret_cast<const bf16x8*>(&w[i]);
+  const int wave = threadIdx.x / WAVE;
+  const int wpb = blockDim.x / WAVE;
+  const bool has_w = w != nullptr;
+  const int D8 = D / NORM_VEC;
+  constexpr int NR = NC > 0 ? NC : 1;
+
+  float sw[NR][NORM_VEC], sb[NR][NORM_VEC];
+  bf16x8 wv[NR];
+  #pragma unroll
+  for (int c = 0; c < NR; ++c) {
     #pragma unroll
-    for (int j = 0; j < VEC; ++j) {
-      float g = bf2f(gv.v[j]);
-      float xh = (bf2f(xv.v[j]) - m) * r;
-      float gw = w ? g * bf2f(wv.v[j]) : g;
-      sum_gw += gw;
-      sum_gwx += gw * xh;
+    for (int j = 0; j < NORM_VEC; ++j) { sw[c][j] = 0.f; sb[c][j] = 0.f; }
+  }
+
+  for (long row = (long)blockIdx.x * wpb + wave; row < rows;
+       row += (long)gridDim.x * wpb) {
+    const T* grow = grad + row * D;
+    const T* xrow = x + row * D;
+    T* dxrow = dx + row * D;
+    const float m = RMS ? 0.f : mean[row];
+    const float r = rstd[row];
+    float sum_gw = 0.f, sum_gwx = 0.f;
+    if constexpr (NC > 0) {
+      bf16x8 gv[NR], xv[NR];
+      #pragma unroll
+      for (int c = 0; c < NC; ++c) {
+        const int i = lane * NORM_VEC + c * NORM_CSTRIDE;
+        if (i < D) {
+          gv[c] = *reinterpret_cast<const bf16x8*>(&grow[i]);
+          xv[c] = *reinterpret_cast<const bf16x8*>(&xrow[i]);
+          if (has_w) wv[c] = *reinterpret_cast<const bf16x8*>(&w[i]);
+        }
+      }
+      #pragma unroll
+      for (int c = 0; c < NC; ++c)
+        if (lane * NORM_VEC + c * NORM_CSTRIDE < D)
+          norm_row_sums<RMS>(gv[c], xv[c], wv[c], has_w, m, r, sum_gw,
+                             sum_gwx);
+      sum_gw = wave_sum(sum_gw) / D;
+      sum_gwx = wave_sum(sum_gwx) / D;
+      #pragma unroll
+      for (int c = 0; c < NC; ++c) { norm_opaque(gv[c]); norm_opaque(xv[c]); }
+      #pragma unroll
+      for (int c = 0; c < NC; ++c) {
+        const int i = lane * NORM_VEC + c * NORM_CSTRIDE;
+        if (i < D)
+          *reinterpret_cast<bf16x8*>(&dxrow[i]) = norm_row_dx<RMS>(
+              gv[c], xv[c], wv[c], has_w, m, r, sum_gw, sum_gwx, sw[c],
+              sb[c]);
+      }
+    } else {
+      for (int i = lane * NORM_VEC; i < D; i += NORM_CSTRIDE) {
+        bf16x8 gv = *reinterpret_cast<const bf16x8*>(&grow[i]);
+        bf16x8 xv = *reinterpret_cast<const bf16x8*>(&xrow[i]);
+        if (has_w) wv[0] = *reinterpret_cast<const bf16x8*>(&w[i]);
+        norm_row_sums<RMS>(gv, xv, wv[0], has_w, m, r, sum_gw, sum_gwx);
+      }
+      sum_gw = wave_sum(sum_gw) / D;
+      sum_gwx = wave_sum(sum_gwx) / D;
+      for (int i = lane * NORM_VEC; i < D; i += NORM_CSTRIDE) {
+        bf16x8 gv = *reinterpret_cast<const bf16x8*>(&grow[i]);
+        bf16x8 xv = *reinterpret_cast<const bf16x8*>(&xrow[i]);
+        if (has_w) wv[0] = *reinterpret_cast<const bf16x8*>(&w[i]);
+        float tw[NORM_VEC], tb[NORM_VEC];
+        #pragma unroll
+        for (int j = 0; j < NORM_VEC; ++j) { tw[j] = 0.f; tb[j] = 0.f; }
+        *reinterpret_cast<bf16x8*>(&dxrow[i]) = norm_row_dx<RMS>(
+            gv, xv, wv[0], has_w, m, r, sum_gw, sum_gwx, tw, tb);
+        #pragma unroll
+        for (int j = 0; j < NORM_VEC; ++j) {
+          atomicAdd(&red[norm_red_slot(i, j, D8)], tw[j]);
+          if (!RMS) atomicAdd(&red[D + norm_red_slot(i, j, D8)], tb[j]);
+        }
+      }
     }
   }
-  sum_gw = wave_sum(sum_gw) / D;
-  sum_gwx = wave_sum(sum_gwx) / D;
-  for (int i = lane * VEC; i < D; i += WAVE * VEC) {
-    bf16x8 gv = *reinterpret_cast<const bf16x8*>(&grow[i]);
-    bf16x8 xv = *reinterpret_cast<const bf16x8*>(&xrow[i]);
-    bf16x8 wv;
-    if (w) wv = *reinterpret_cast<const bf16x8*>(&w[i]);
-    bf16x8 dxv;
+
+  if constexpr (NC > 0) {
     #pragma unroll
-    for (int j = 0; j < VEC; ++j) {
-      float g = bf2f(gv.v[j]);
-      float xh = (bf2f(xv.v[j]) - m) * r;
-      float gw = w ? g * bf2f(wv.v[j]) : g;
-      float v = RMS ? r * (gw - xh * sum_gwx)
-                    : r * (gw - sum_gw - xh * sum_gwx);
-      dxv.v[j] = f2bf(v);
+    for (int c = 0; c < NC; ++c) {
+      const int i = lane * NORM_VEC + c * NORM_CSTRIDE;
+      if (i < D) {
+        #pragma unroll
+        for (int j = 0; j < NORM_VEC; ++j) {
+          atomicAdd(&red[norm_red_slot(i, j, D8)], sw[c][j]);
+          if (!RMS) atomicAdd(&red[D + norm_red_slot(i, j, D8)], sb[c][j]);
+        }
+      }
     }
-    *reinterpret_cast<bf16x8*>(&dxrow[i]) = dxv;
-  }
-}
-
-template <typename T, bool RMS>
-__global__ void norm_param_grads_kernel(const T* __restrict__ grad,
-                                        const T* __restrict__ x,
-                                        const float* __restrict__ mean,
-                                        const float* __restrict__ rstd,
-                                        float* __restrict__ dw,
-                                        float* __restrict__ db,
-                                        int rows, int D, int rows_per_blk) {
-  const int col0 = (blockIdx.x * blockDim.x + threadIdx.x) * 8;
-  if (col0 >= D) return;
-  const int r0 = blockIdx.y * rows_per_blk;
-  const int r1 = min(r0 + rows_per_blk, rows);
-  float sw[8] = {0, 0, 0, 0, 0, 0, 0, 0};
-  float sb[8] = {0, 0, 0, 0, 0, 0, 0, 0};
-  for (int r = r0; r < r1; ++r) {
-    const bf16x8 g8 = *reinterpret_cast<const bf16x8*>(
-        &grad[(long)r * D + col0]);
-    const bf16x8 x8 = *reinterpret_cast<const bf16x8*>(
-        &x[(long)r * D + col0]);
-    const float m = RMS ? 0.f : mean[r];
-    const float rs = rstd[r];
-    #pragma unroll
-    for (int u = 0; u < 8; ++u) {
-      float g = bf2f(g8.v[u]);
-      sw[u] += g * (bf2f(x8.v[u]) - m) * rs;
-      sb[u] += g;
-    }
-  }
-  #pragma unroll
-  for (int u = 0; u < 8; ++u) {
-    atomicAdd(&dw[col0 + u], sw[u]);
-    atomicAdd(&db[col0 + u], sb[u]);
-  }
-}
-
-template <typename T, bool RMS>
-__global__ void norm_param_grads_scalar_kernel(const T* __restrict__ grad,
-                                               const T* __restrict__ x,
-                                               const float* __restrict__ mean,
-                                               const float* __restrict__ rstd,
-                                               float* __restrict__ dw,
-                                               float* __restrict__ db,
-                                               int rows, int D,
-                                               int rows_per_blk) {
-  const int col = blockIdx.x * blockDim.x + threadIdx.x;
-  if (col >= D) return;
-  const int r0 = blockIdx.y * rows_per_blk;
-  const int r1 = min(r0 + rows_per_blk, rows);
-  float sw = 0.f, sb = 0.f;
-  #pragma unroll 8
-  for (int r = r0; r < r1; ++r) {
-    float g = bf2f(grad[(long)r * D + col]);
-    float m = RMS ? 0.f : mean[r];
-    float xh = (bf2f(x[(long)r * D + col]) - m) * rstd[r];
-    sw += g * xh;
-    sb += g;
-  }
-  atomicAdd(&dw[col], sw);
-  atomicAdd(&db[col], sb);
-}
-
-static bool lnpg_scalar() {
-  static int v = [] {
-    const char* e = getenv("EASYDIST_LNPG");
-    return (e && std::string(e) == "vector") ? 0 : 1;
-  }();
-  return v;
+  }
+  __syncthreads();
+  for (int c = threadIdx.x; c < nred; c += blockDim.x) {
+    const int stat = c / D, col = c % D;
+    atomicAdd(&dwb[c], red[stat * D + norm_red_slot(col & ~7, col & 7, D8)]);
+  }
 }
 
 #include <torch/extension.h>
@@ -277,6 +311,37 @@
   return {out, mean, rstd};
 }
 
+template <bool RMS>
+static at::Tensor norm_bwd_launch(const at::Tensor& grad, const at::Tensor& x,
+                                  const float* mean, const at::Tensor& rstd,
+                                  const std::optional<at::Tensor>& w,
+                                  at::Tensor& dx) {
+  const int D = x.size(-1);
+  const long rows = x.numel() / D;
+  const int nstat = RMS ? 1 : 2;
+  auto dwb = at::zeros({nstat, D}, x.options().dtype(at::kFloat));
+  const size_t lds = (size_t)nstat * D * sizeof(float);
+  TORCH_CHECK(lds <= 65536, "norm backward: feature dim too wide for the "
+              "LDS column accumulator");
+  const int max_blocks =
+      at::cuda::getCurrentDeviceProperties()->multiProcessorCount;
+  const int wpb = NORM_BWD_THREADS / WAVE;
+  const long want = std::max<long>(1, (rows + wpb - 1) / wpb);
+  dim3 block(NORM_BWD_THREADS), grid((unsigned)std::min<long>(want, max_blocks));
+  auto stream = at::cuda::getCurrentCUDAStream();
+  const int nc = (D + NORM_CSTRIDE - 1) / NORM_CSTRIDE;
+#define NORM_BWD_LAUNCH(NC)                                                  \
+  hipLaunchKernelGGL((norm_bwd_kernel<bf16, RMS, NC>), grid, block, lds,     \
+      stream, (const bf16*)grad.data_ptr(), (const bf16*)x.data_ptr(), mean, \
+      rstd.data_ptr<float>(), w ? (const bf16*)w->data_ptr() : nullptr,      \
+      (bf16*)dx.data_ptr(), dwb.data_ptr<float>(), (int)rows, D)
+  if (nc == 1) NORM_BWD_LAUNCH(1);
+  else if (nc == 2) NORM_BWD_LAUNCH(2);
+  else NORM_BWD_LAUNCH(0);
+#undef NORM_BWD_LAUNCH
+  return dwb;
+}
+
 std::tuple<at::Tensor, at::Tensor, at::Tensor>
 layer_norm_bwd(const at::Tensor& grad, const at::Tensor& x,
                const at::Tensor& mean, const at::Tensor& rstd,
@@ -288,41 +353,10 @@
   TORCH_CHECK(mean.numel() == x.numel() / x.size(-1));
   TORCH_CHECK(x.scalar_type() == at::kBFloat16,
               "layer_norm_bwd kernel: bf16 only (fp32 falls back to aten)");
-  const int D = x.size(-1);
-  const long rows = x.numel() / D;
   auto dx = at::empty_like(x);
-  auto dwf = at::zeros({D}, x.options().dtype(at::kFloat));
-  auto dbf = at::zeros({D}, x.options().dtype(at::kFloat));
-  auto stream = at::cuda::getCurrentCUDAStream();
-  const int WPB = 4;
-  dim3 block(WAVE * WPB), grid((rows + WPB - 1) / WPB);
-  hipLaunchKernelGGL((norm_bwd_kernel<bf16, false>), grid, block, 0, stream,
-      (const bf16*)grad.data_ptr(), (const bf16*)x.data_ptr(),
-      mean.data_ptr<float>(), rstd.data_ptr<float>(),
-      w ? (const bf16*)w->data_ptr() : nullptr, (bf16*)dx.data_ptr(),
-      dwf.data_ptr<float>(), dbf.data_ptr<float>(), rows, D);
-  const int gx = (D + 511) / 512;
-  int rows_per_blk = 256;
-  while ((long)gx * ((rows + rows_per_blk - 1) / rows_per_blk) > 1024)
-    rows_per_blk *= 2;
-  dim3 gblock(64), ggrid(gx, (rows + rows_per_blk - 1) / rows_per_blk);
-  if (lnpg_scalar()) {
-    const int rpb2 = 256;
-    dim3 sb2(256), sg2((D + 255) / 256, (rows + rpb2 - 1) / rpb2);
-    hipLaunchKernelGGL((norm_param_grads_scalar_kernel<bf16, false>), sg2,
-        sb2, 0, stream, (const bf16*)grad.data_ptr(),
-        (const bf16*)x.data_ptr(), mean.data_ptr<float>(),
-        rstd.data_ptr<float>(), dwf.data_ptr<float>(),
-        dbf.data_ptr<float>(), rows, D, rpb2);
-    auto dtype0 = at::kFloat;
-    return {dx, dwf.to(dtype0), dbf.to(dtype0)};
-  }
-  hipLaunchKernelGGL((norm_param_grads_kernel<bf16, false>), ggrid, gblock, 0,
-      stream, (const bf16*)grad.data_ptr(), (const bf16*)x.data_ptr(),
-      mean.data_ptr<float>(), rstd.data_ptr<float>(), dwf.data_ptr<float>(),
-      dbf.data_ptr<float>(), rows, D, rows_per_blk);
-  auto dtype = at::kFloat;
-  return {dx, dwf.to(dtype), dbf.to(dtype)};
+  auto dwb = norm_bwd_launch<false>(grad, x, mean.data_ptr<float>(), rstd, w,
+                                    dx);
+  return {dx, dwb[0], dwb[1]};
 }
 
 std::tuple<at::Tensor, at::Tensor>
@@ -360,28 +394,7 @@
   check_affine(x, w, std::nullopt);
   TORCH_CHECK(grad.sizes() == x.sizes() && grad.is_contiguous());
   TORCH_CHECK(x.scalar_type() == at::kBFloat16, "rms_norm_bwd: bf16 only");
-  const int D = x.size(-1);
-  const long rows = x.numel() / D;
   auto dx = at::empty_like(x);
-  auto dwf = at::zeros({D}, x.options().dtype(at::kFloat));
-  auto dbf = at::zeros({D}, x.options().dtype(at::kFloat));
-  auto stream = at::cuda::getCurrentCUDAStream();
-  const int WPB = 4;
-  dim3 block(WAVE * WPB), grid((rows + WPB - 1) / WPB);
-  hipLaunchKernelGGL((norm_bwd_kernel<bf16, true>), grid, block, 0, stream,
-      (const bf16*)grad.data_ptr(), (const bf16*)x.data_ptr(), nullptr,
-      rstd.data_ptr<float>(), w ? (const bf16*)w->data_ptr() : nullptr,
-      (bf16*)dx.data_ptr(), dwf.data_ptr<float>(), dbf.data_ptr<float>(),
-      rows, D);
-  const int gx = (D + 511) / 512;
-  int rows_per_blk = 256;
-  while ((long)gx * ((rows + rows_per_blk - 1) / rows_per_blk) > 1024)
-    rows_per_blk *= 2;
-  dim3 gblock(64), ggrid(gx, (rows + rows_per_blk - 1) / rows_per_blk);
-  hipLaunchKernelGGL((norm_param_grads_kernel<bf16, true>), ggrid, gblock, 0,
-      stream, (const bf16*)grad.data_ptr(), (const bf16*)x.data_ptr(),
-      nullptr, rstd.data_ptr<float>(), dwf.data_ptr<float>(),
-      dbf.data_ptr<float>(), rows, D, rows_per_blk);
-  auto dtype = at::kFloat;
-  return {dx, dwf.to(dtype)};
-}
+  auto dwb = norm_bwd_launch<true>(grad, x, nullptr, rstd, w, dx);
+  return {dx, dwb[0]};
+}
diff --git a/easydist_amd/ops/csrc/optim_kernels.hip b/easydist_amd/ops/csrc/optim_kernels.hip
--- a/easydist_amd/ops/csrc/optim_kernels.hip
+++ b/easydist_amd/ops/csrc/optim_kernels.hip
@@ -14,7 +14,8 @@
   float* out_p;
   float* out_ea;
   float* out_eas;
-  int tensor_idx;
+  const float* in_step;
+  float* out_step;
   int n;
 };
 
@@ -81,13 +82,13 @@
 
 __global__ void fused_adam_kernel(const AdamChunk* __restrict__ chunks,
                                   int n_chunks, int g_bf16,
-                                  const float* __restrict__ steps,
                                   float lr, float beta1, float beta2,
                                   float weight_decay, float eps) {
   const int c = blockIdx.x;
   if (c >= n_chunks) return;
   const AdamChunk ch = chunks[c];
-  const float step = steps[ch.tensor_idx] + 1.f;
+  const float step = *ch.in_step + 1.f;
+  if (ch.out_step && threadIdx.x == 0) *ch.out_step = step;
   const float bc1 = 1.f - __powf(beta1, step);
   const float bc2 = 1.f - __powf(beta2, step);
   const float inv_bc1 = 1.f / bc1;
@@ -129,13 +130,6 @@
   }
 }
 
-__global__ void bump_steps_kernel(const float* const* __restrict__ in_steps,
-                                  float* const* __restrict__ out_steps,
-                                  int n) {
-  int i = blockIdx.x * blockDim.x + threadIdx.x;
-  if (i < n) out_steps[i][0] = in_steps[i][0] + 1.f;
-}
-
 std::tuple<std::vector<at::Tensor>, std::vector<at::Tensor>,
            std::vector<at::Tensor>, std::vector<at::Tensor>>
 fused_adam_step(std::vector<at::Tensor> params, std::vector<at::Tensor> grads,
@@ -144,8 +138,9 @@
                 std::vector<at::Tensor> steps, double lr, double beta1,
                 double beta2, double weight_decay, double eps) {
   const int T = params.size();
-  std::vector<at::Tensor> out_p, out_ea, out_eas, out_steps;
+  std::vector<at::Tensor> out_p, out_ea, out_eas, out_steps, steps_f;
   out_p.reserve(T); out_ea.reserve(T); out_eas.reserve(T);
+  out_steps.reserve(T); steps_f.reserve(T);
   const bool g_bf16 = !grads.empty()
       && grads[0].scalar_type() == at::kBFloat16;
   for (int t = 0; t < T; ++t) {
@@ -157,19 +152,16 @@
     out_p.push_back(at::empty_like(params[t]));
     out_ea.push_back(at::empty_like(exp_avgs[t]));
     out_eas.push_back(at::empty_like(exp_avg_sqs[t]));
-    out_steps.push_back(at::empty_like(steps[t]));
-  }
-  auto steps_flat = at::empty({T}, params[0].options());
-  {
-    std::vector<at::Tensor> svec;
-    for (auto& s : steps) svec.push_back(s.reshape({1}).to(at::kFloat));
-    at::cat_out(steps_flat, svec, 0);
+    TORCH_CHECK(steps[t].numel() == 1, "step counters are one-element");
+    steps_f.push_back(steps[t].scalar_type() == at::kFloat
+                          ? steps[t] : steps[t].to(at::kFloat));
+    out_steps.push_back(at::empty_like(steps_f[t]));
   }
 
   std::vector<AdamChunk> chunks;
   for (int t = 0; t < T; ++t) {
     long n = params[t].numel();
-    for (long off = 0; off < n; off += CHUNK_ELEMS) {
+    for (long off = 0; off == 0 || off < n; off += CHUNK_ELEMS) {
       AdamChunk c;
       c.p = params[t].data_ptr<float>() + off;
       c.g = g_bf16 ? (const void*)((const bf16*)grads[t].data_ptr() + off)
@@ -179,7 +171,8 @@
       c.out_p = out_p[t].data_ptr<float>() + off;
       c.out_ea = out_ea[t].data_ptr<float>() + off;
       c.out_eas = out_eas[t].data_ptr<float>() + off;
-      c.tensor_idx = t;
+      c.in_step = steps_f[t].data_ptr<float>();
+      c.out_step = off == 0 ? out_steps[t].data_ptr<float>() : nullptr;
       c.n = (int)std::min<long>(CHUNK_ELEMS, n - off);
       chunks.push_back(c);
     }
@@ -197,11 +190,12 @@
                                 bytes, hipMemcpyHostToDevice, stream));
   hipLaunchKernelGGL(fused_adam_kernel, dim3(chunks.size()), dim3(256), 0,
       stream, (const AdamChunk*)st.dev.data_ptr(), (int)chunks.size(),
-      (int)g_bf16, steps_flat.data_ptr<float>(), (float)lr, (float)beta1,
+      (int)g_bf16, (float)lr, (float)beta1,
       (float)beta2, (float)weight_decay, (float)eps);
   staging_finish(g_pool, bytes, key, capturing, stream);
   for (int t = 0; t < T; ++t)
-    out_steps[t] = steps[t] + 1;
+    if (steps[t].scalar_type() != at::kFloat)
+      out_steps[t] = out_steps[t].to(steps[t].scalar_type());
   return {out_p, out_ea, out_eas, out_steps};
 }
 
```

Result: no change. 734.4 samples/sec, median of 6 (+0.9%).
